# lucasbrynte/gasfm

Measured on AMD Instinct MI355X. Metric: GAT-stack edges/sec (fwd+bwd) on cam/point scene graph; 1/2/4/8 MI355X, higher is better.
Workload: dtype fp32; 1 GPU; config 4: m=1000 cameras, n=200000 points, E=4001638 projections, 12-block GraphAttnSfMNet (learning_euc widths) fwd+bwd; cameras=1000, points=200000, edges=4001638, blocks=12, parallelism=single GPU

## Files before the change

gasfm_amd/_native.py:

```python
import ctypes
import threading
import os

import numpy as np
import torch

from . import _abi
from .build import LIB

_C = _abi.constants
GASFM_OK, GASFM_ERR_INVALID, GASFM_ERR_OOM, GASFM_ERR_HIP, GASFM_ERR_UNSUPPORTED = (
    _C[k] for k in ("GASFM_OK", "GASFM_ERR_INVALID", "GASFM_ERR_OOM", "GASFM_ERR_HIP", "GASFM_ERR_UNSUPPORTED"))

_vp = ctypes.c_void_p
_i32 = ctypes.c_int32
_i64 = ctypes.c_int64

_SIGS = _abi.functions

_lib = None


def lib():
    global _lib
    if _lib is None:
        path = os.environ.get("GASFM_LIB") or LIB
        if not os.path.exists(path):
            raise ImportError(
                f"gasfm native library not built: {path} missing. Run `python -m gasfm_amd.build` "
                "(hipcc --offload-arch=gfx950). There is no CPU fallback.")
        L = ctypes.CDLL(path)
        for name, (res, args) in _SIGS.items():
            fn = getattr(L, name)
            fn.restype = res
            fn.argtypes = args
        _lib = L
    return _lib


def exported_symbols():
    return list(_SIGS)


def check(status, what):
    if status == GASFM_OK:
        return
    msg = lib().gasfm_last_error().decode(errors="replace")
    if status == GASFM_ERR_OOM:
        raise torch.OutOfMemoryError(f"{what}: {msg}")
    raise RuntimeError(f"{what} failed (status {status}): {msg}")


def _p(t):
    return None if t is None else ctypes.c_void_p(t.data_ptr())


_RAW_STREAM = getattr(torch._C, "_cuda_getCurrentRawStream", None)


def _stream(t):
    if _RAW_STREAM is not None and t.device.index is not None:
        return ctypes.c_void_p(_RAW_STREAM(t.device.index))
    return ctypes.c_void_p(torch.cuda.current_stream(t.device).cuda_stream)


def _enum(prefix):
    return {k[len(prefix):].lower(): v for k, v in _C.items() if k.startswith(prefix) and k != prefix + "COUNT"}


KERNELS = _enum("GASFM_K_")
TUNING = _enum("GASFM_TUNE_")


def dispatch_counts():
    n = _C["GASFM_K_COUNT"]
    buf = (_i64 * n)()
    lib().gasfm_dispatch_counts(buf, n)
    return {k: int(buf[i]) for k, i in KERNELS.items()}


def dispatch_reset():
    lib().gasfm_dispatch_reset()


def tuning_get(key):
    return float(lib().gasfm_tuning_get(TUNING[key]))


def tuning_set(key, value):
    check(lib().gasfm_tuning_set(TUNING[key], float(value)), "gasfm_tuning_set")


class tuned:

    def __init__(self, **kv):
        self.kv = kv

    def __enter__(self):
        self.prev = {k: tuning_get(k) for k in self.kv}
        for k, v in self.kv.items():
            tuning_set(k, v)
        return self

    def __exit__(self, *exc):
        for k, v in self.prev.items():
            tuning_set(k, v)
        return False


class dispatch_record:

    def __enter__(self):
        self.start = dispatch_counts()
        return self

    def __exit__(self, *exc):
        end = dispatch_counts()
        self.counts = {k: end[k] - self.start[k] for k in end}
        return False


def build_csr(key, n):
    key = np.ascontiguousarray(key, dtype=np.int32)
    E = key.shape[0]
    ptr = np.empty(n + 1, dtype=np.int32)
    perm = np.empty(max(E, 1), dtype=np.int32)
    st = lib().gasfm_build_csr(key.ctypes.data_as(_vp), E, n, ptr.ctypes.data_as(_vp),
                               perm.ctypes.data_as(_vp))
    check(st, "gasfm_build_csr")
    return ptr, perm[:E]


def plan_work(seg_ptr, max_piece, all_partial=False):
    seg_ptr = np.ascontiguousarray(seg_ptr, dtype=np.int32)
    N = seg_ptr.shape[0] - 1
    ni, nc, ns = _i32(0), _i32(0), _i32(0)
    L = lib()
    L.gasfm_plan_work(seg_ptr.ctypes.data_as(_vp), N, max_piece, int(all_partial), None,
                      ctypes.byref(ni), None, ctypes.byref(nc), ctypes.byref(ns))
    items = np.empty((max(ni.value, 1), 4), dtype=np.int32)
    comb = np.empty((max(nc.value, 1), 4), dtype=np.int32)
    ni2, nc2 = _i32(ni.value), _i32(nc.value)
    st = L.gasfm_plan_work(seg_ptr.ctypes.data_as(_vp), N, max_piece, int(all_partial),
                           items.ctypes.data_as(_vp), ctypes.byref(ni2), comb.ctypes.data_as(_vp),
                           ctypes.byref(nc2), ctypes.byref(ns))
    check(st, "gasfm_plan_work")
    return items[:ni2.value], comb[:nc2.value], ns.value


def attn_fwd(XL, XR, att, bias, perm, items, n_items, H, C, slope, finalize, out, seg_max, seg_sum, part=None,
             ldStat=None, lanes=False):
    ldStat = H if ldStat is None else ldStat
    fn = lib().gasfm_gat_attn_fwd_lanes if lanes else lib().gasfm_gat_attn_fwd
    st = fn(
        _p(XL), XL.stride(0), _p(XR), XR.stride(0), _p(att), _p(bias), _p(perm), _p(items), n_items, H, C,
        slope, int(finalize), _p(out), out.stride(0) if out is not None else 0, _p(seg_max), _p(seg_sum), ldStat,
        _p(part), _stream(XL))
    check(st, "gasfm_gat_attn_fwd")


def attn_combine(combine, n_combine, H, C, part, bias, finalize, out, seg_max, seg_sum, ldOut=None, ldStat=None):
    ldOut = out.stride(0) if ldOut is None else ldOut
    ldStat = H if ldStat is None else ldStat
    st = lib().gasfm_gat_attn_combine(_p(combine), n_combine, H, C, _p(part), _p(bias), int(finalize), _p(out),
                                      ldOut, _p(seg_max), _p(seg_sum), ldStat, _stream(part))
    check(st, "gasfm_gat_attn_combine")


def attn_bwd_waves(n_items, H, C):
    return lib().gasfm_gat_attn_bwd_waves(n_items, H, C)


def attn_bwd(XL, XR, att, bias, perm, items, n_items, H, C, slope, out, seg_max, seg_sum, gout, dXL, dXR,
             part_dxr, datt_part, xl_by_position=False, lanes=False):
    fn = lib().gasfm_gat_attn_bwd_lanes if lanes else lib().gasfm_gat_attn_bwd
    st = fn(
        _p(XL), XL.stride(0), _p(XR), XR.stride(0), _p(att), _p(bias), _p(perm), _p(items), n_items, H, C,
        slope, _p(out), out.stride(0), _p(seg_max), _p(seg_sum), _p(gout), gout.stride(0), _p(dXL),
        dXL.stride(0), _p(dXR), dXR.stride(0), _p(part_dxr), _p(datt_part), int(xl_by_position), _stream(dXL))
    check(st, "gasfm_gat_attn_bwd")


def attn_bwd_combine(combine, n_combine, HC, part_dxr, dXR):
    st = lib().gasfm_gat_attn_bwd_combine(_p(combine), n_combine, HC, _p(part_dxr), _p(dXR), dXR.stride(0),
                                          _stream(dXR))
    check(st, "gasfm_gat_attn_bwd_combine")


def attn_bwd_combine2(combine, n_combine, HC, part_a, out_a, part_b, out_b):
    st = lib().gasfm_gat_attn_bwd_combine2(_p(combine), n_combine, HC, _p(part_a), _p(out_a), out_a.stride(0),
                                           _p(part_b), _p(out_b), out_b.stride(0), _stream(out_a))
    check(st, "gasfm_gat_attn_bwd_combine2")


_COUNTERS = {}
_COUNTER_POOL = 1 << 16


def _counters(device, n):
    n = max(1, int(n))
    if n > _COUNTER_POOL:
        raise ValueError(f"colsum counters: {n} requested, pool holds {_COUNTER_POOL}")
    c = _COUNTERS.get(device)
    if c is None:
        c = [torch.zeros(_COUNTER_POOL, dtype=torch.int32, device=device), 0]
        _COUNTERS[device] = c
    pool, at = c
    if at + n > _COUNTER_POOL:
        at = 0
    c[1] = at + n
    return pool[at:at + n]


def colsum(A, out=None):
    assert A.dim() == 2 and A.stride(1) == 1 and A.dtype == torch.float32
    rows, cols = A.shape
    if out is None:
        out = torch.empty(cols, dtype=torch.float32, device=A.device)
    L = lib()
    ws = torch.empty(int(L.gasfm_colsum_ws_floats(rows, cols)), dtype=torch.float32, device=A.device)
    cnt = _counters(A.device, L.gasfm_colsum_counters(cols))
    st = L.gasfm_colsum(_p(A), rows, cols, max(A.stride(0), cols), _p(ws), _p(out), _p(cnt), _stream(out))
    check(st, "gasfm_colsum")
    return out


def colsum_tall_ok(A):
    return (A.dim() == 2 and A.is_contiguous() and A.dtype == torch.float32
            and bool(lib().gasfm_colsum_tall_ok(A.shape[1])))


def colsum_tall(A, out=None):
    rows, cols = A.shape
    if out is None:
        out = torch.empty(cols, dtype=torch.float32, device=A.device)
    L = lib()
    ws = torch.empty(max(1, int(L.gasfm_colsum_tall_ws_floats(rows, cols))), dtype=torch.float32, device=A.device)
    cnt = _counters(A.device, 1)
    st = L.gasfm_colsum_tall(_p(A), rows, cols, _p(ws), _p(out), _p(cnt), _stream(out))
    check(st, "gasfm_colsum_tall")
    return out


def colsum_ranges(A, row_ptr, w=None, out=None):
    if not (A.is_cuda and A.dim() == 2 and A.dtype == torch.float32 and (A.shape[1] == 1 or A.stride(1) == 1)):
        raise ValueError("colsum_ranges: A must be a 2-D fp32 CUDA tensor with unit column stride")
    rows, cols = A.shape
    if cols < 1:
        raise ValueError("colsum_ranges: A has no columns")
    if row_ptr.dtype != torch.int32 or row_ptr.dim() != 1 or row_ptr.numel() < 1 or not row_ptr.is_contiguous() \
            or row_ptr.device != A.device:
        raise ValueError("colsum_ranges: row_ptr must be a contiguous int32 vector on A's device")
    n_ranges = row_ptr.numel() - 1
    if w is not None and not (w.dtype == torch.float64 and w.dim() == 1 and w.numel() == rows and w.is_contiguous()
                              and w.device == A.device):
        raise ValueError("colsum_ranges: w must be a contiguous fp64 vector with one entry per row of A")
    if out is None:
        out = torch.empty((n_ranges, cols), dtype=torch.float64, device=A.device)
    elif not (out.dtype == torch.float64 and tuple(out.shape) == (n_ranges, cols) and out.is_contiguous()
              and out.device == A.device):
        raise ValueError(f"colsum_ranges: out must be a contiguous fp64 [{n_ranges}, {cols}] tensor")
    ld = max(A.stride(0), cols) if rows > 1 else cols
    st = lib().gasfm_colsum_ranges(_p(A), ld, cols, _p(row_ptr), n_ranges, _p(w), _p(out), _stream(out))
    check(st, "gasfm_colsum_ranges")
    return out



_DEFER_FWD = False
_PENDING = {}
_SEEN = {}
_PENDING_LOCK = threading.Lock()


def defer_token(*targets):
    if _DEFER_FWD and all(t is None or t.is_leaf for t in targets):
        return tuple(t for t in targets if t is not None) or True
    return False


class deferring_param_grads:

    def __init__(self, enabled):
        self.enabled = bool(enabled)

    def __enter__(self):
        global _DEFER_FWD
        self.prev, _DEFER_FWD = _DEFER_FWD, self.enabled
        return self

    def __exit__(self, *exc):
        global _DEFER_FWD
        _DEFER_FWD = self.prev
        return False


def param_colsum(A, defer):
    task = torch._C._current_graph_task_id() if defer else -1
    if task < 0:
        return colsum(A)
    if isinstance(defer, tuple) and any(t.grad is not None for t in defer):
        return colsum(A)
    if isinstance(defer, tuple):
        with _PENDING_LOCK:
            seen = _SEEN.setdefault(task, {})
            again = any(seen.get(id(t), id(defer)) != id(defer) for t in defer)
            for t in defer:
                seen.setdefault(id(t), id(defer))
        if again and os.environ.get("GASFM_DEBUG_DEFER"):
            print("param_colsum: repeated targets", [tuple(t.shape) for t in defer], flush=True)
        if again:
            _flush_param_colsums(task, final=False)
            return colsum(A)
    assert A.dim() == 2 and A.stride(1) == 1 and A.dtype == torch.float32
    rows, cols = A.shape
    L = lib()
    out = torch.empty(cols, dtype=torch.float32, device=A.device)
    ws = torch.empty(int(L.gasfm_colsum_ws_floats(rows, cols)), dtype=torch.float32, device=A.device)
    job = (A, ws, out, rows, cols, max(A.stride(0), cols), torch.cuda.current_stream(A.device))
    with _PENDING_LOCK:
        jobs = _PENDING.get(task)
        first = jobs is None
        if first:
            jobs = _PENDING[task] = []
        jobs.append(job)
    if first:
        torch.autograd.Variable._execution_engine.queue_callback(lambda: _flush_param_colsums(task))
    return out


def _flush_param_colsums(task, final=True):
    with _PENDING_LOCK:
        jobs = _PENDING.pop(task, [])
        if final:
            _SEEN.pop(task, None)
    if not jobs:
        return
    stream = jobs[0][6]
    assert all(j[6] == stream for j in jobs), "param_colsum: jobs queued on several streams"
    n = len(jobs)
    L = lib()
    arr = lambda ty, xs: (ty * n)(*xs)
    A = arr(ctypes.c_void_p, [j[0].data_ptr() for j in jobs])
    ws = arr(ctypes.c_void_p, [j[1].data_ptr() for j in jobs])
    out = arr(ctypes.c_void_p, [j[2].data_ptr() for j in jobs])
    rows = arr(ctypes.c_int64, [j[3] for j in jobs])
    cols = arr(ctypes.c_int32, [j[4] for j in jobs])
    ld = arr(ctypes.c_int64, [j[5] for j in jobs])
    dev = jobs[0][0].device
    cnt = _counters(dev, L.gasfm_colsum_multi_counters(n, cols))
    st = L.gasfm_colsum_multi(n, A, rows, cols, ld, ws, out, _p(cnt), ctypes.c_void_p(stream.cuda_stream))
    check(st, "gasfm_colsum_multi")


def _req(t, name, cols=None):
    if not t.is_cuda or t.dtype != torch.float32 or not t.is_contiguous():
        raise TypeError(f"{name}: expected a contiguous float32 CUDA tensor (no CPU fallback)")
    if cols is not None and t.shape[-1] != cols:
        raise ValueError(f"{name}: expected {cols} columns, got {tuple(t.shape)}")


def edge_part_floats(which, E, n_items=0):
    return lib().gasfm_edge_part_floats(which, E, n_items)


def edge_prologue_fwd(P, ln_w, ln_b, eps, W, b, Y, pos=None, W2=None, b2=None):
    _req(P, "P", 32)
    st = lib().gasfm_edge_prologue_fwd(_p(P), P.shape[0], _p(ln_w), _p(ln_b), eps, _p(W), _p(W2), _p(b), _p(b2),
                                       _p(Y), Y.stride(0), _p(pos), _stream(P))
    check(st, "gasfm_edge_prologue_fwd")


def _rows32(t, name):
    if not t.is_cuda or t.dtype != torch.float32 or t.dim() != 2 or t.shape[1] != 32 or t.stride(1) != 1 \
            or (t.shape[0] > 1 and t.stride(0) < 32):
        raise TypeError(f"{name}: expected [rows, 32] float32 CUDA rows with unit column stride")
    return t.stride(0) if t.shape[0] > 1 else 32


def edge_epilogue_fwd(P, P0, cam, pt, ln_w, ln_b, eps, Wp, bp, Sp, Sv, Sg, scale, out):
    _req(P, "P", 32)
    for t, n in ((Sp, "Sp"), (Sg, "Sg"), (Wp, "Wp")):
        _req(t, n)
    ldSv = _rows32(Sv, "Sv")
    st = lib().gasfm_edge_epilogue_fwd(_p(P), _p(P0), _p(cam), _p(pt), P.shape[0], _p(ln_w), _p(ln_b), eps, _p(Wp),
                                       Wp.shape[1], _p(bp), _p(Sp), _p(Sv), ldSv, _p(Sg), scale, _p(out),
                                       _stream(P))
    check(st, "gasfm_edge_epilogue_fwd")


def edge_epilogue_bwd(items, n_items, dPo, P, P0, ln_w, ln_b, eps, Wp, scale, dSv, part_dsv, dP0, part_w):
    _req(dPo, "dP'", 32)
    st = lib().gasfm_edge_epilogue_bwd(_p(items), n_items, _p(dPo), _p(P), _p(P0), _p(ln_w), _p(ln_b), eps, _p(Wp),
                                       Wp.shape[1], scale, _p(dSv), _p(part_dsv), _p(dP0), _p(part_w), _stream(dPo))
    check(st, "gasfm_edge_epilogue_bwd")


def edge_prologue_bwd(dXL, P, dRes, ln_w, ln_b, eps, W, Wp, scale, dP, part, W2=None, dXLc=None):
    _req(P, "P", 32)
    st = lib().gasfm_edge_prologue_bwd(_p(dXL), dXL.stride(0), _p(P), _p(dRes), P.shape[0], _p(ln_w), _p(ln_b), eps,
                                       _p(W), _p(W2), _p(Wp), Wp.shape[1] if Wp is not None else 0, scale, _p(dP),
                                       _p(part), _p(dXLc), dXLc.stride(0) if dXLc is not None else 0, _stream(P))
    check(st, "gasfm_edge_prologue_bwd")


def edge_cam_fwd(P, ln_w, ln_b, eps, Wpt, bpt, Wc, bc, XLp, pos, XR, att, bias, slope, plan_items, n_items,
                 finalize, out, seg_max, seg_sum, part, ldStat=4):
    _req(P, "P", 32)
    ldXR = _rows32(XR, "XR")
    st = lib().gasfm_edge_cam_fwd(_p(P), _p(ln_w), _p(ln_b), eps, _p(Wpt), _p(bpt), _p(Wc), _p(bc), _p(XLp),
                                  XLp.stride(0), _p(pos), _p(XR), ldXR, _p(att), _p(bias), slope, _p(plan_items),
                                  n_items, int(finalize), _p(out), out.stride(0) if out is not None else 0,
                                  _p(seg_max), _p(seg_sum), ldStat, _p(part), _stream(P))
    check(st, "gasfm_edge_cam_fwd")


def _ld_stat(seg_max):
    return seg_max.stride(0) if seg_max is not None else 4


def edge_seam_fwd(Pb, P0, pt, lnw_b, lnb_b, eps_b, Wp, bp, Sp, Sv, Sg, scale, Pout, ln_w, ln_b, eps, Wpt, bpt, Wc, bc,
                  XLp, pos, XR, att, bias, slope, plan_items, n_items, finalize, out, seg_max, seg_sum, part):
    _req(Pb, "Pb", 32)
    ldXR = _rows32(XR, "XR")
    ldSv = _rows32(Sv, "Sv")
    st = lib().gasfm_edge_seam_fwd(_p(Pb), _p(P0), _p(pt), _p(lnw_b), _p(lnb_b), eps_b, _p(Wp), Wp.stride(0), _p(bp),
                                   _p(Sp), _p(Sv), ldSv, _p(Sg), scale, _p(Pout), _p(ln_w), _p(ln_b), eps, _p(Wpt),
                                   _p(bpt), _p(Wc), _p(bc), _p(XLp), XLp.stride(0), _p(pos), _p(XR), ldXR, _p(att),
                                   _p(bias), slope, _p(plan_items), n_items, int(finalize), _p(out),
                                   out.stride(0) if out is not None else 0, _p(seg_max), _p(seg_sum), _ld_stat(seg_max),
                                   _p(part), _stream(Pb))
    check(st, "gasfm_edge_seam_fwd")


def edge0_seam_fwd(P, pt, lna_w, lna_b, lnb_w, lnb_b, eps0, Wp, bp, Wsk, bsk, Sp, Sv, Sg, scale, Pout, ln_w, ln_b, eps,
                   Wpt, bpt, Wc, bc, XLp, pos, XR, att, bias, slope, plan_items, n_items, finalize, out, seg_max,
                   seg_sum, part):
    _req(P, "P", 2)
    ldXR = _rows32(XR, "XR")
    ldSv = _rows32(Sv, "Sv")
    st = lib().gasfm_edge0_seam_fwd(_p(P), _p(pt), _p(lna_w), _p(lna_b), _p(lnb_w), _p(lnb_b), eps0, _p(Wp), _p(bp),
                                    _p(Wsk), _p(bsk), _p(Sp), _p(Sv), ldSv, _p(Sg), scale, _p(Pout), _p(ln_w), _p(ln_b),
                                    eps, _p(Wpt), _p(bpt), _p(Wc), _p(bc), _p(XLp), XLp.stride(0), _p(pos), _p(XR),
                                    ldXR, _p(att), _p(bias), slope, _p(plan_items), n_items, int(finalize), _p(out),
                                    out.stride(0) if out is not None else 0, _p(seg_max), _p(seg_sum),
                                    _ld_stat(seg_max), _p(part), _stream(P))
    check(st, "gasfm_edge0_seam_fwd")


def edge_cam_pbwd_part_shape(n_items, dwp_cols=0):
    L = lib()
    return int(L.gasfm_edge_cam_pbwd_part_rows(n_items)), int(L.gasfm_edge_cam_pbwd_part_cols()) + 32 * dwp_cols


def edge_cam_pbwd(P, ln_w, ln_b, eps, Wpt, Wc, bc, Wp, scale, XR, att, bias, slope, out, seg_max, seg_sum, gout,
                  plan_items, n_items, dXLp, dRes, dP, dXR, part_dxr, part, ldStat=4, epi=None, dwp=None):
    _req(P, "P", 32)
    ldXR = _rows32(XR, "XR")
    We = dSv = part_dsv = dP0 = None
    scale_e, ldWe = 0.0, 0
    if epi is not None:
        We, scale_e, dSv, part_dsv, dP0 = epi
        _req(dSv, "dSv", 32)
        if dP0 is not None:
            _req(dP0, "dP0", 2)
        ldWe = We.stride(0)
    P0, ldWpo = None, 0
    if dwp is not False and dwp is not None:
        P0 = dwp if isinstance(dwp, torch.Tensor) else None
        ldWpo = 34 if P0 is not None else 32
    if P0 is not None:
        _req(P0, "P0", 2)
    st = lib().gasfm_edge_cam_pbwd_ex(_p(P), _p(ln_w), _p(ln_b), eps, _p(Wpt), _p(Wc), _p(bc), _p(Wp),
                                      Wp.stride(0) if Wp is not None else 0, scale, _p(XR), ldXR, _p(att), _p(bias),
                                      slope, _p(out), out.stride(0), _p(seg_max), _p(seg_sum), ldStat, _p(gout),
                                      gout.stride(0), _p(plan_items), n_items, _p(dXLp), dXLp.stride(0), _p(dRes),
                                      _p(dP), _p(dXR), dXR.stride(0), _p(part_dxr), _p(part), part.stride(0), _p(We),
                                      ldWe, scale_e, _p(dSv), _p(part_dsv), _p(dP0), _p(P0), ldWpo, _stream(P))
    check(st, "gasfm_edge_cam_pbwd")


def segment_rowsum(items, n_items, perm, X, scale, out, part):
    st = lib().gasfm_segment_rowsum(_p(items), n_items, _p(perm), _p(X), X.stride(0), scale, _p(out), _p(part),
                                    _stream(X))
    check(st, "gasfm_segment_rowsum")


def sos_width_ok(d_in, d_out):
    return bool(lib().gasfm_sos_width_ok(int(d_in), int(d_out)))


def sos_row_tile(n_cols):
    return int(lib().gasfm_sos_row_tile(int(n_cols)))


def sos_segment_sum(plan, X, scale=1.0, mean=False, mask=None):
    _req(X, "sos_segment_sum X")
    D = X.shape[1]
    out = torch.zeros((plan.num_targets, D), dtype=torch.float32, device=X.device)
    if plan.n_items == 0 or X.shape[0] == 0:
        return out
    if mask is not None:
        _req(mask, "sos_segment_sum mask", D)
    part = torch.empty((plan.n_part_rows, D), dtype=torch.float32, device=X.device) if plan.n_part_rows else None
    st = lib().gasfm_sos_segment_sum(_p(plan.items), plan.n_items, _p(plan.perm), _p(X), X.stride(0), _p(mask),
                                     0 if mask is None else mask.stride(0), D, float(scale),
                                     _p(plan.seg_ptr) if mean else None, _p(out), _p(part), _stream(X))
    check(st, "gasfm_sos_segment_sum")
    if part is not None:
        if plan.n_l1:
            attn_bwd_combine(plan.combine_l1, plan.n_l1, D, part, part)
        if plan.n_combine:
            attn_bwd_combine(plan.combine, plan.n_combine, D, part, out)
    return out


def sos_edge_fwd(X, W, cam, pt, S, V, cmean, R, relu, out=None):
    _req(X, "sos_edge_fwd X")
    E, d_in = X.shape
    d_out = W.shape[0]
    for t, name, cols in ((W, "W", d_in), (S, "S", d_out), (V, "V", d_out)):
        _req(t, "sos_edge_fwd " + name, cols)
    Y = torch.empty((E, d_out), dtype=torch.float32, device=X.device) if out is None else out
    _req(Y, "sos_edge_fwd out", d_out)
    if Y.shape[0] != E:
        raise ValueError(f"sos_edge_fwd out: {Y.shape[0]} rows, expected {E}")
    if E == 0:
        return Y
    if cam.shape[0] != E or pt.shape[0] != E or cam.dtype != torch.int32 or pt.dtype != torch.int32:
        raise ValueError("sos_edge_fwd: cam / pt must be int32 [E]")
    if cmean is not None:
        _req(cmean, "sos_edge_fwd cmean", d_out)
    if R is not None:
        _req(R, "sos_edge_fwd R", d_out)
    st = lib().gasfm_sos_edge_fwd(_p(X), X.stride(0), _p(W), E, d_in, d_out, _p(cam), _p(pt), _p(S), _p(V),
                                  _p(cmean), _p(R), 0 if R is None else R.stride(0), int(bool(relu)), _p(Y),
                                  _stream(X))
    check(st, "gasfm_sos_edge_fwd")
    return Y


def sos_edge_dx(dY, Ym, W, cam, pt, Ac, Bp, E, d_in, out=None):
    dev = cam.device
    dX = torch.empty((E, d_in), dtype=torch.float32, device=dev) if out is None else out
    _req(dX, "sos_edge_dx out", d_in)
    if dX.shape[0] != E or cam.shape[0] != E or pt.shape[0] != E or (dY is not None and dY.shape[0] != E):
        raise ValueError("sos_edge_dx: row counts differ")
    if E == 0:
        return dX
    d_out = 0 if dY is None else dY.shape[1]
    for t, name, cols in ((dY, "dY", None), (Ym, "Ym", d_out), (W, "W", d_in), (Ac, "Ac", d_in), (Bp, "Bp", d_in)):
        if t is not None:
            _req(t, "sos_edge_dx " + name, cols)
    st = lib().gasfm_sos_edge_dx(_p(dY), _p(Ym), _p(W), E, d_in, d_out, _p(cam), _p(pt), _p(Ac), _p(Bp), _p(dX),
                                 _stream(dX))
    check(st, "gasfm_sos_edge_dx")
    return dX


def sos_edge_dw(dY, Ym, X):
    _req(dY, "sos_edge_dw dY")
    _req(X, "sos_edge_dw X")
    E, d_out = dY.shape
    d_in = X.shape[1]
    if E == 0:
        return torch.zeros((d_out, d_in), dtype=torch.float32, device=dY.device)
    if Ym is not None:
        _req(Ym, "sos_edge_dw Ym", d_out)
    L = lib()
    splits = int(L.gasfm_sos_dw_splits(E, d_in, d_out))
    part = torch.empty((splits, d_out * d_in), dtype=torch.float32, device=dY.device)
    st = L.gasfm_sos_edge_dw(_p(dY), _p(Ym), _p(X), X.stride(0), E, d_in, d_out, splits, _p(part), _stream(dY))
    check(st, "gasfm_sos_edge_dw")
    if splits == 1:
        return part.view(d_out, d_in)
    return colsum(part).view(d_out, d_in)


def edge0_part_rows(which, E, n_items=0):
    return lib().gasfm_edge0_part_rows(which, E, n_items)


def edge0_prologue_fwd(P, ln_w, ln_b, eps, W0, b0, XL, pos=None):
    _req(P, "P", 2)
    st = lib().gasfm_edge0_prologue_fwd(_p(P), P.shape[0], _p(ln_w), _p(ln_b), eps, _p(W0), _p(b0), _p(XL),
                                        _p(pos), _stream(P))
    check(st, "gasfm_edge0_prologue_fwd")


def edge0_prologue_fwd_rows(P, ln_w, ln_b, eps, W0, b0, XL, perm):
    _req(P, "P", 2)
    if perm.dtype != torch.int32 or perm.numel() != P.shape[0] or perm.device != P.device:
        raise ValueError("edge0_prologue_fwd_rows: perm must be int32 [E] on P's device")
    st = lib().gasfm_edge0_prologue_fwd_rows(_p(P), P.shape[0], _p(ln_w), _p(ln_b), eps, _p(W0), _p(b0), _p(XL),
                                             _p(perm), _stream(P))
    check(st, "gasfm_edge0_prologue_fwd_rows")


def edge0_epilogue_fwd(P, cam, pt, lna_w, lna_b, lnb_w, lnb_b, eps, Wp, bp, Wsk, bsk, Sp, Sv, Sg, scale, out):
    _req(P, "P", 2)
    for t, n in ((Sp, "Sp"), (Sg, "Sg")):
        _req(t, n)
    ldSv = _rows32(Sv, "Sv")
    st = lib().gasfm_edge0_epilogue_fwd(_p(P), _p(cam), _p(pt), P.shape[0], _p(lna_w), _p(lna_b), _p(lnb_w),
                                        _p(lnb_b), eps, _p(Wp), _p(bp), _p(Wsk), _p(bsk), _p(Sp), _p(Sv), ldSv,
                                        _p(Sg), scale, _p(out), _stream(P))
    check(st, "gasfm_edge0_epilogue_fwd")


def edge0_epilogue_bwd(items, n_items, dPo, P, lna_w, lna_b, lnb_w, lnb_b, eps, Wp, Wsk, scale, dSv, part_dsv, aux,
                       part):
    _req(dPo, "dP'", 32)
    st = lib().gasfm_edge0_epilogue_bwd(_p(items), n_items, _p(dPo), _p(P), _p(lna_w), _p(lna_b), _p(lnb_w),
                                        _p(lnb_b), eps, _p(Wp), _p(Wsk), scale, _p(dSv), _p(part_dsv), _p(aux),
                                        _p(part), _stream(dPo))
    check(st, "gasfm_edge0_epilogue_bwd")


def edge0_prologue_bwd(dXL, P, aux, ln_w, ln_b, eps, W0, dP, part):
    _req(dXL, "dXL0", 8)
    st = lib().gasfm_edge0_prologue_bwd(_p(dXL), _p(P), _p(aux), P.shape[0], _p(ln_w), _p(ln_b), eps, _p(W0),
                                        _p(dP), _p(part), _stream(P))
    check(st, "gasfm_edge0_prologue_bwd")


def node_part_rows(N, n_out, residual):
    return lib().gasfm_node_part_rows(N, n_out, int(residual))


def node_ln_linear_fwd(X, ln_w, ln_b, eps, W, b, residual, Y):
    _req(X, "X")
    N, n_in = X.shape
    st = lib().gasfm_node_ln_linear_fwd(_p(X), N, n_in, _p(ln_w), _p(ln_b), eps, _p(W), _p(b), W.shape[0],
                                        int(residual), _p(Y), Y.stride(0), _stream(X))
    check(st, "gasfm_node_ln_linear_fwd")


def node_ln_linear_bwd(dY, X, ln_w, ln_b, eps, W, residual, dX, part):
    _req(dY, "dY", W.shape[0])
    _req(X, "X")
    N, n_in = X.shape
    st = lib().gasfm_node_ln_linear_bwd(_p(dY), _p(X), N, n_in, _p(ln_w), _p(ln_b), eps, _p(W), W.shape[0],
                                        int(residual), _p(dX), _p(part), _stream(X))
    check(st, "gasfm_node_ln_linear_bwd")


def gvec_bwd_chunks(N):
    return lib().gasfm_gvec_bwd_chunks(N)


def gvec_fwd(x, ln_w, ln_b, eps, W, b, res, y):
    _req(x, "x")
    _req(W, "W")
    st = lib().gasfm_gvec_fwd(_p(x), W.shape[1], _p(ln_w), _p(ln_b), eps, _p(W), _p(b), W.shape[0], _p(res), _p(y),
                              _stream(x))
    check(st, "gasfm_gvec_fwd")


def gvec_bwd(dy, x, ln_w, ln_b, eps, W, resid, dx, dW, db, dgam, dbet, part):
    _req(dy, "dy")
    st = lib().gasfm_gvec_bwd(_p(dy), _p(x), W.shape[1], _p(ln_w), _p(ln_b), eps, _p(W), W.shape[0], int(resid),
                              _p(dx), _p(dW), _p(db), _p(dgam), _p(dbet), _p(part), _stream(x))
    check(st, "gasfm_gvec_bwd")


def point_tail_part_shape(N, has_prev):
    cols = ctypes.c_int32(0)
    rows = lib().gasfm_point_tail_part_shape(N, int(has_prev), ctypes.byref(cols))
    return rows, cols.value


def point_hub_part_shape(N, which, has_res):
    cols = ctypes.c_int32(0)
    rows = lib().gasfm_point_hub_part_shape(N, int(which), int(has_res), ctypes.byref(cols))
    return rows, cols.value


def point_tail_fwd(prev, agg, Wp, bp, ln_w, ln_b, eps, Wm, bm, out):
    _req(agg, "agg", 32)
    if prev is not None:
        _req(prev, "prev", 64)
    st = lib().gasfm_point_tail_fwd(_p(prev), _p(agg), agg.shape[0], _p(Wp), _p(bp), _p(ln_w), _p(ln_b), eps,
                                    _p(Wm), _p(bm), _p(out), _stream(agg))
    check(st, "gasfm_point_tail_fwd")


def point_tail_bwd(dout, prev, agg, Wp, bp, ln_w, ln_b, eps, Wm, dx, dagg, part):
    _req(dout, "dout", 64)
    _req(agg, "agg", 32)
    if prev is not None:
        _req(prev, "prev", 64)
    st = lib().gasfm_point_tail_bwd(_p(dout), _p(prev), _p(agg), agg.shape[0], _p(Wp), _p(bp), _p(ln_w), _p(ln_b),
                                    eps, _p(Wm), _p(dx), _p(dagg), _p(part), _stream(agg))
    check(st, "gasfm_point_tail_bwd")


def point_hub_fwd(X, eps, gA, bA, WA, SA, WB, bB, XL, gC, bC, WC, bWC, WD, bD, XR):
    _req(X, "X", 64)
    st = lib().gasfm_point_hub_fwd(_p(X), X.shape[0], eps, _p(gA), _p(bA), _p(WA), _p(SA), _p(WB), _p(bB), _p(XL),
                                   _p(gC), _p(bC), _p(WC), _p(bWC), _p(WD), _p(bD), _p(XR), _stream(X))
    check(st, "gasfm_point_hub_fwd")


def point_tail_hub_fwd(prev, agg, Wp, bp, ln_w, ln_b, eps, Wm, bm, out, eps_h, gA, bA, WA, SA, WB, bB, XL, gC, bC,
                       WC, bWC, WD, bD, XR):
    _req(agg, "agg", 32)
    _req(out, "out", 64)
    if prev is not None:
        _req(prev, "prev", 64)
    st = lib().gasfm_point_tail_hub_fwd(_p(prev), _p(agg), agg.shape[0], _p(Wp), _p(bp), _p(ln_w), _p(ln_b), eps,
                                        _p(Wm), _p(bm), _p(out), eps_h, _p(gA), _p(bA), _p(WA), _p(SA), _p(WB), _p(bB),
                                        _p(XL), _p(gC), _p(bC), _p(WC), _p(bWC), _p(WD), _p(bD), _p(XR), _stream(agg))
    check(st, "gasfm_point_tail_hub_fwd")


def point_hub_bwd(X, eps, gA, bA, WA, WB, gC, bC, WC, bWC, WD, dSA, dXL, dXR, dRes, dX, part_a, part_c):
    _req(X, "X", 64)
    _req(dSA, "dSA", 32)
    _req(dXL, "dXL", 64)
    _req(dXR, "dXR", 32)
    if dRes is not None:
        _req(dRes, "dRes", 64)
    st = lib().gasfm_point_hub_bwd(_p(X), X.shape[0], eps, _p(gA), _p(bA), _p(WA), _p(WB), _p(gC), _p(bC), _p(WC),
                                   _p(bWC), _p(WD), _p(dSA), _p(dXL), _p(dXR), _p(dRes), _p(dX), _p(part_a),
                                   _p(part_c), _stream(X))
    check(st, "gasfm_point_hub_bwd")


def embed2_fwd(X, W, b, Y):
    _req(X, "values", 2)
    _req(Y, "P", 2)
    st = lib().gasfm_embed2_fwd(_p(X), X.shape[0], _p(W), _p(b), _p(Y), _stream(X))
    check(st, "gasfm_embed2_fwd")


def embed2_bwd(X, dY, defer=False):
    _req(X, "values", 2)
    _req(dY, "dP", 2)
    E = X.shape[0]
    rows = lib().gasfm_embed2_part_rows(E)
    if rows == 0:
        tot = torch.zeros(6, dtype=torch.float32, device=X.device)
    else:
        part = torch.empty((rows, 6), dtype=torch.float32, device=X.device)
        st = lib().gasfm_embed2_bwd(_p(X), _p(dY), E, _p(part), _stream(X))
        check(st, "gasfm_embed2_bwd")
        tot = param_colsum(part, defer)
    return tot[:4].view(2, 2), tot[4:]


def point_head_part_shape(N, which):
    cols = ctypes.c_int32(0)
    rows = lib().gasfm_point_head_part_shape(N, int(which), ctypes.byref(cols))
    return rows, cols.value


def _head_weights(W1, b1, W2, b2, W3, b3=None):
    shapes = ((W1, (64, 64)), (b1, (64,)), (W2, (64, 64)), (b2, (64,)), (W3, (3, 64))) + \
        (((b3, (3,)),) if b3 is not None else ())
    for t, shape in shapes:
        if tuple(t.shape) != shape or not t.is_contiguous() or t.dtype != torch.float32:
            raise ValueError(f"point head: weight {tuple(t.shape)} is not a contiguous fp32 {shape}")


def point_head_fwd(P, W1, b1, W2, b2, W3, b3, out):
    _req(P, "P", 64)
    _head_weights(W1, b1, W2, b2, W3, b3)
    N = P.shape[0]
    if tuple(out.shape) != (4, N) or not out.is_contiguous():
        raise ValueError("point_head_fwd: out must be a contiguous [4, N]")
    st = lib().gasfm_point_head_fwd(_p(P), N, _p(W1), _p(b1), _p(W2), _p(b2), _p(W3), _p(b3), _p(out), _stream(P))
    check(st, "gasfm_point_head_fwd")


def point_head_bwd(P, W1, b1, W2, b2, W3, dout, dP, part_a, part_b):
    _req(P, "P", 64)
    _req(dP, "dP", 64)
    _head_weights(W1, b1, W2, b2, W3)
    N = P.shape[0]
    if tuple(dout.shape) != (4, N) or not dout.is_contiguous():
        raise ValueError("point_head_bwd: dout must be a contiguous [4, N]")
    for part, which in ((part_a, 0), (part_b, 1)):
        if tuple(part.shape) != point_head_part_shape(N, which) or not part.is_contiguous():
            raise ValueError("point_head_bwd: partial buffer of the wrong shape")
    st = lib().gasfm_point_head_bwd(_p(P), N, _p(W1), _p(b1), _p(W2), _p(b2), _p(W3), _p(dout), _p(dP),
                                    _p(part_a), _p(part_b), _stream(P))
    check(st, "gasfm_point_head_bwd")


def view_tail_part_cols(D):
    return lib().gasfm_view_tail_part_cols(D)


def view_hub_part_cols(D):
    return lib().gasfm_view_hub_part_cols(D)


def view_scratch(m, D, device):
    return torch.empty(max(1, int(lib().gasfm_view_scratch_floats(m, D))), dtype=torch.float32, device=device)


def view_tail_fwd(prev, agg, Wp, bp, ln_w, ln_b, eps, bm, x, xb, h, rs, scratch):
    _req(agg, "agg", 32)
    D = x.shape[1]
    if prev is not None:
        _req(prev, "prev", D)
    st = lib().gasfm_view_tail_fwd(_p(prev), _p(agg), agg.shape[0], D, _p(Wp), _p(bp), _p(ln_w), _p(ln_b), eps,
                                   _p(bm), _p(x), _p(xb), _p(h), _p(rs), _p(scratch), _stream(agg))
    check(st, "gasfm_view_tail_fwd")


def view_tail_bwd(dv, dh, x, rs, agg, Wp, ln_w, ln_b, dx, dagg, part, scratch):
    D = x.shape[1]
    for t, n in ((dv, "dv"), (dh, "dh"), (x, "x")):
        _req(t, n, D)
    _req(agg, "agg", 32)
    st = lib().gasfm_view_tail_bwd(_p(dv), _p(dh), _p(x), _p(rs), _p(agg), agg.shape[0], D, _p(Wp), _p(ln_w),
                                   _p(ln_b), _p(dx), _p(dagg), _p(part), _p(scratch), _stream(agg))
    check(st, "gasfm_view_tail_bwd")


def view_hub_fwd(v, eps, gC, bC, Wv, gA, bA, Wa, ba, Wr, br, sv, t, xr, rs, scratch):
    _req(v, "v")
    ldo = _rows32(sv, "sv")
    if _rows32(xr, "xr") != ldo:
        raise ValueError("view_hub_fwd: sv and xr need the same row stride")
    st = lib().gasfm_view_hub_fwd(_p(v), v.shape[0], v.shape[1], eps, _p(gC), _p(bC), _p(Wv), _p(gA), _p(bA), _p(Wa),
                                  _p(ba), _p(Wr), _p(br), _p(sv), _p(t), _p(xr), ldo, _p(rs), _p(scratch), _stream(v))
    check(st, "gasfm_view_hub_fwd")


def view_chain_ok(m, D):
    return bool(lib().gasfm_view_chain_ok(m, D))


def _vc_scratch(m, D, device):
    return torch.empty(max(1, int(lib().gasfm_view_chain_scratch_floats(m, D))), dtype=torch.float32, device=device)


def view_chain_tail_fwd(prev, agg, Wp, bp, ln_w, ln_b, eps, Wm, bm, view, x, h, rs):
    _req(agg, "agg", 32)
    m, D = view.shape
    for t, n in ((view, "view"), (x, "x"), (h, "h"), (Wm, "Wm"), (Wp, "Wp")) + (((prev, "prev"),) if prev is not None else ()):
        _req(t, n)
    st = lib().gasfm_view_chain_tail_fwd(_p(prev), _p(agg), m, D, _p(Wp), _p(bp), _p(ln_w), _p(ln_b), eps, _p(Wm),
                                         _p(bm), _p(view), _p(x), _p(h), _p(rs), _stream(agg))
    check(st, "gasfm_view_chain_tail_fwd")


def view_chain_hub_fwd(v, eps, Wl, bl, gC, bC, Wv, gA, bA, Wa, ba, Wr, br, XL, sv, t, xr, rs):
    _req(v, "v")
    ldo = _rows32(sv, "sv")
    if _rows32(xr, "xr") != ldo:
        raise ValueError("view_chain_hub_fwd: sv and xr need the same row stride")
    for a, n in ((Wl, "Wl"), (Wv, "Wv"), (Wa, "Wa"), (XL, "XL")):
        _req(a, n)
    st = lib().gasfm_view_chain_hub_fwd(_p(v), v.shape[0], v.shape[1], eps, _p(Wl), _p(bl), _p(gC), _p(bC), _p(Wv),
                                        _p(gA), _p(bA), _p(Wa), _p(ba), _p(Wr), _p(br), _p(XL), _p(sv), _p(t), _p(xr),
                                        ldo, _p(rs), _stream(v))
    check(st, "gasfm_view_chain_hub_fwd")


def view_chain_hub_bwd(v, rs, gC, bC, Wv, gA, bA, Wa, t, Wr, Wl, dsv, dxr, dxl, dres, dacc, dWl, part):
    _req(v, "v")
    m, D = v.shape
    for a, n, w in ((t, "t", 32), (dsv, "dsv", 32), (dxr, "dxr", 32), (dxl, "dxl", D), (dacc, "dacc", D),
                    (dWl, "dWl", D)):
        _req(a, n, w)
    if dres is not None:
        _req(dres, "dres", D)
    scratch = _vc_scratch(m, D, v.device)
    st = lib().gasfm_view_chain_hub_bwd(_p(v), _p(rs), m, D, _p(gC), _p(bC), _p(Wv), _p(gA), _p(bA), _p(Wa), _p(t),
                                        _p(Wr), _p(Wl), _p(dsv), _p(dxr), _p(dxl), _p(dres), _p(dacc), _p(dWl),
                                        _p(part), _p(scratch), _stream(v))
    check(st, "gasfm_view_chain_hub_bwd")


def view_chain_tail_bwd(dv, x, h, rs, agg, Wp, ln_w, ln_b, Wm, dh, dWm, dx, dagg, part):
    m, D = x.shape
    for a, n in ((dv, "dv"), (x, "x"), (h, "h"), (dh, "dh"), (dx, "dx"), (dWm, "dWm")):
        _req(a, n, D)
    _req(agg, "agg", 32)
    scratch = _vc_scratch(m, D, x.device)
    cnt = _counters(x.device, lib().gasfm_view_chain_counters(m))
    st = lib().gasfm_view_chain_tail_bwd(_p(dv), _p(x), _p(h), _p(rs), _p(agg), m, D, _p(Wp), _p(ln_w), _p(ln_b),
                                         _p(Wm), _p(dh), _p(dWm), _p(dx), _p(dagg), _p(part), _p(scratch), _p(cnt),
                                         _stream(x))
    check(st, "gasfm_view_chain_tail_bwd")


def view_hub_bwd(v, rs, gC, bC, Wv, gA, bA, Wa, t, Wr, dsv, dxr, dxl, dacc, part, scratch, dres=None):
    _req(v, "v")
    D = v.shape[1]
    for a, n, w in ((t, "t", 32), (dsv, "dsv", 32), (dxr, "dxr", 32), (dxl, "dxl", D), (dacc, "dacc", D)):
        _req(a, n, w)
    if dres is not None:
        _req(dres, "dres", D)
    st = lib().gasfm_view_hub_bwd(_p(v), _p(rs), v.shape[0], D, _p(gC), _p(bC), _p(Wv), _p(gA), _p(bA), _p(Wa),
                                  _p(t), _p(Wr), _p(dsv), _p(dxr), _p(dxl), _p(dres), _p(dacc), _p(part),
                                  _p(scratch), _stream(v))
    check(st, "gasfm_view_hub_bwd")


def pose_fwd(x, P):
    if not x.is_cuda or x.dtype != torch.float32 or x.stride(1) != 1:
        raise TypeError("pose x: expected a float32 CUDA tensor with unit column stride (no CPU fallback)")
    check(lib().gasfm_pose_fwd(_p(x), x.stride(0), x.shape[0], _p(P), _stream(x)), "gasfm_pose_fwd")


def pose_bwd(x, dP, dx):
    _req(dP, "dP")
    check(lib().gasfm_pose_bwd(_p(x), x.stride(0), x.shape[0], _p(dP), _p(dx), dx.stride(0), _stream(x)),
          "gasfm_pose_bwd")


def _i32vec(t, name):
    if not t.is_cuda or t.dtype != torch.int32 or t.dim() != 1 or not t.is_contiguous():
        raise TypeError(f"{name}: expected a contiguous int32 CUDA vector")


def _edge_args(name, cam, pt, vals, P, X, csr=None, seg=None, scene_of=None, f32=()):
    vecs = [(cam, "cam"), (pt, "pt")]
    if csr is not None:
        vecs += [(csr[0], "cam_ptr"), (csr[1], "pt_ptr")] + ([] if csr[2] is None else [(csr[2], "perm")])
    if scene_of is not None:
        vecs += [(scene_of[0], "scene_of_cam"), (scene_of[1], "scene_of_pt")]
    for t, tname in vecs:
        _i32vec(t, f"{name}: {tname}")
    for t, tname, cols in ((vals, "vals", 2), (P, "P", 12), (X, "pts3D", None)) + tuple(f32):
        _req(t, f"{name}: {tname}", cols)
    if X.dim() != 2 or X.shape[0] != 4 or P.dim() != 2 or vals.dim() != 2:
        raise ValueError(f"{name}: expected P [m, 12], pts3D [4, n] and vals [E, 2]")
    E, m, n = cam.shape[0], P.shape[0], X.shape[1]
    if pt.shape[0] != E or vals.shape[0] != E:
        raise ValueError(f"{name}: expected pts3D [4, n] and E-long cam / pt / values")
    if csr is not None and (csr[0].shape[0] != m + 1 or csr[1].shape[0] != n + 1
                            or (csr[2] is not None and csr[2].shape[0] != E)):
        raise ValueError(f"{name}: CSR shapes do not match m / n / E")
    if scene_of is not None and (scene_of[0].shape[0] != m or scene_of[1].shape[0] != n):
        raise ValueError(f"{name}: scene map shapes do not match m / n")
    if seg is not None:
        eoff, S = seg
        if not eoff.is_cuda or eoff.dtype != torch.int32 or not eoff.is_contiguous() or eoff.numel() != S + 1:
            raise TypeError(f"{name}: eoff must be a contiguous int32 [S + 1] CUDA tensor")
    return E, m, n


def _grad_args(dloss, dP, dX, n, tot=None):
    return ((dloss, "dloss", None), (dP, "dP", 12), (dX, "dX", n)) + (() if tot is None else ((tot, "tot", None),))


def esfm_part_rows(E):
    return lib().gasfm_esfm_part_rows(E)


def esfm_fwd(cam, pt, vals, P, X, margin, hinge_w, hinge, part):
    E, _, n = _edge_args("esfm_fwd", cam, pt, vals, P, X)
    st = lib().gasfm_esfm_fwd(_p(cam), _p(pt), _p(vals), E, _p(P), _p(X), n, margin, hinge_w, int(hinge), _p(part),
                              _stream(X))
    check(st, "gasfm_esfm_fwd")


def esfm_bwd(cptr, pptr, perm, cam, pt, vals, P, X, margin, hinge_w, hinge, equalize, valid_only, dloss, tot, dP,
             dX, E_norm=None):
    E, m, n = _edge_args("esfm_bwd", cam, pt, vals, P, X, csr=(cptr, pptr, perm),
                         f32=_grad_args(dloss, dP, dX, X.shape[-1], tot))
    E_norm = E if E_norm is None else int(E_norm)
    st = lib().gasfm_esfm_bwd(_p(cptr), m, _p(pptr), _p(perm), _p(cam), _p(pt), _p(vals), E, E_norm, _p(P), _p(X), n,
                              margin, hinge_w, int(hinge), int(equalize), int(valid_only), _p(dloss), _p(tot), _p(dP),
                              _p(dX), _stream(X))
    check(st, "gasfm_esfm_bwd")


def esfm_seg_fwd(cam, pt, vals, eoff, weight, P, X, margin, hinge_w, hinge):
    S = int(weight.numel())
    _, _, n = _edge_args("esfm_seg_fwd", cam, pt, vals, P, X, seg=(eoff, S), f32=((weight, "weight", None),))
    dev = X.device
    part = torch.empty((lib().gasfm_esfm_seg_part_rows(S), 2), dtype=torch.float32, device=dev)
    tot = torch.empty((S, 2), dtype=torch.float32, device=dev)
    loss = torch.empty(1, dtype=torch.float32, device=dev)
    st = lib().gasfm_esfm_seg_fwd(_p(cam), _p(pt), _p(vals), _p(eoff), S, _p(weight), _p(P), _p(X), n, margin, hinge_w,
                                  int(hinge), _p(part), _p(tot), _p(loss), _stream(X))
    check(st, "gasfm_esfm_seg_fwd")
    return loss, tot


def esfm_seg_bwd(cptr, pptr, perm, cam, pt, vals, eoff, scene_of_cam, scene_of_pt, weight, P, X, margin, hinge_w,
                 hinge, equalize, valid_only, dloss, tot, dP, dX):
    S = int(weight.numel())
    _, m, n = _edge_args("esfm_seg_bwd", cam, pt, vals, P, X, csr=(cptr, pptr, perm), seg=(eoff, S),
                         scene_of=(scene_of_cam, scene_of_pt),
                         f32=((weight, "weight", None),) + _grad_args(dloss, dP, dX, X.shape[-1], tot))
    st = lib().gasfm_esfm_seg_bwd(_p(cptr), m, _p(pptr), _p(perm), _p(cam), _p(pt), _p(vals), _p(eoff), S,
                                  _p(scene_of_cam), _p(scene_of_pt), _p(weight), _p(P), _p(X), n, margin, hinge_w,
                                  int(hinge), int(equalize), int(valid_only), _p(dloss), _p(tot), _p(dP), _p(dX),
                                  _stream(X))
    check(st, "gasfm_esfm_seg_bwd")


def ose_fwd(cam, pt, vals, P, X, w_reg):
    E, _, n = _edge_args("ose_fwd", cam, pt, vals, P, X)
    part = torch.empty((lib().gasfm_ose_part_rows(E), 1), dtype=torch.float32, device=X.device)
    st = lib().gasfm_ose_fwd(_p(cam), _p(pt), _p(vals), E, _p(P), _p(X), n, w_reg, _p(part), _stream(X))
    check(st, "gasfm_ose_fwd")
    return part


def ose_bwd(cptr, pptr, perm, cam, pt, vals, P, X, w_reg, dloss, dP, dX):
    E, m, n = _edge_args("ose_bwd", cam, pt, vals, P, X, csr=(cptr, pptr, perm),
                         f32=_grad_args(dloss, dP, dX, X.shape[-1]))
    st = lib().gasfm_ose_bwd(_p(cptr), m, _p(pptr), _p(perm), _p(cam), _p(pt), _p(vals), E, _p(P), _p(X), n, w_reg,
                             _p(dloss), _p(dP), _p(dX), _stream(X))
    check(st, "gasfm_ose_bwd")


def ose_seg_fwd(cam, pt, vals, eoff, weight, P, X, w_reg):
    S = int(weight.numel())
    _, _, n = _edge_args("ose_seg_fwd", cam, pt, vals, P, X, seg=(eoff, S), f32=((weight, "weight", None),))
    dev = X.device
    part = torch.empty(lib().gasfm_ose_seg_part_rows(S), dtype=torch.float32, device=dev)
    tot = torch.empty(S, dtype=torch.float32, device=dev)
    loss = torch.empty(1, dtype=torch.float32, device=dev)
    st = lib().gasfm_ose_seg_fwd(_p(cam), _p(pt), _p(vals), _p(eoff), S, _p(weight), _p(P), _p(X), n, w_reg, _p(part),
                                 _p(tot), _p(loss), _stream(X))
    check(st, "gasfm_ose_seg_fwd")
    return loss, tot


def ose_seg_bwd(cptr, pptr, perm, cam, pt, vals, eoff, scene_of_cam, scene_of_pt, weight, P, X, w_reg, dloss, dP, dX):
    S = int(weight.numel())
    _, m, n = _edge_args("ose_seg_bwd", cam, pt, vals, P, X, csr=(cptr, pptr, perm), seg=(eoff, S),
                         scene_of=(scene_of_cam, scene_of_pt),
                         f32=((weight, "weight", None),) + _grad_args(dloss, dP, dX, X.shape[-1]))
    st = lib().gasfm_ose_seg_bwd(_p(cptr), m, _p(pptr), _p(perm), _p(cam), _p(pt), _p(vals), _p(eoff), S,
                                 _p(scene_of_cam), _p(scene_of_pt), _p(weight), _p(P), _p(X), n, w_reg, _p(dloss),
                                 _p(dP), _p(dX), _stream(X))
    check(st, "gasfm_ose_seg_bwd")


def reproj_error(cam, pt, xy, P, X, err=None):
    E, _, n = _edge_args("reproj_error", cam, pt, xy, P, X, f32=() if err is None else ((err, "err", None),))
    if err is not None and err.shape[0] != E:
        raise ValueError("reproj_error: expected pts3D [4, n] and E-long cam / pt / xy / err")
    part = torch.empty((esfm_part_rows(E), 2), dtype=torch.float32, device=X.device)
    st = lib().gasfm_reproj_error(_p(cam), _p(pt), _p(xy), E, _p(P), _p(X), n, _p(err), _p(part), _stream(X))
    check(st, "gasfm_reproj_error")
    return part


def reproj_error_seg(cam, pt, xy, eoff, S, P, X):
    _, _, n = _edge_args("reproj_error_seg", cam, pt, xy, P, X, seg=(eoff, S))
    dev = X.device
    part = torch.empty((lib().gasfm_esfm_seg_part_rows(S), 2), dtype=torch.float32, device=dev)
    tot = torch.empty((S, 2), dtype=torch.float32, device=dev)
    st = lib().gasfm_reproj_error_seg(_p(cam), _p(pt), _p(xy), _p(eoff), S, _p(P), _p(X), n, _p(part), _p(tot),
                                      _stream(X))
    check(st, "gasfm_reproj_error_seg")
    return tot


def depth_stats(cam, pt, cam_ptr, pt_ptr, perm, P, X, margin, depth=None):
    E, m, n = cam.shape[0], cam_ptr.shape[0] - 1, pt_ptr.shape[0] - 1
    for t, name in ((cam, "cam"), (pt, "pt"), (cam_ptr, "cam_ptr"), (pt_ptr, "pt_ptr")):
        _i32vec(t, name)
    if perm is not None:
        _i32vec(perm, "perm")
    _req(P, "P", 12), _req(X, "pts3D", n)
    if (X.dim() != 2 or X.shape[0] != 4 or P.dim() != 2 or P.shape[0] != m or pt.shape[0] != E
            or (perm is not None and perm.shape[0] != E) or (depth is not None and depth.shape[0] != E)):
        raise ValueError("depth_stats: expected P [m, 12], pts3D [4, n], cam_ptr [m + 1], pt_ptr [n + 1] and "
                         "E-long cam / pt / perm / depth")
    if depth is not None:
        _req(depth, "depth")
    dev = cam_ptr.device
    cam_neg = torch.empty(m, dtype=torch.int32, device=dev)
    pt_neg = torch.empty(n, dtype=torch.int32, device=dev)
    stats = torch.empty(6, dtype=torch.float64, device=dev)
    L = lib()
    ws = torch.empty(int(L.gasfm_depth_stats_ws_doubles(E)), dtype=torch.float64, device=dev)
    st = L.gasfm_depth_stats(_p(cam), _p(pt), E, _p(cam_ptr), m, _p(pt_ptr), _p(perm), n, _p(P), _p(X),
                             float(margin), _p(depth), _p(cam_neg), _p(pt_neg), _p(ws), _p(stats), _stream(cam_ptr))
    check(st, "gasfm_depth_stats")
    return cam_neg, pt_neg, stats


def _depth_args(a, b, name):
    _req(a, "depths"), _req(b, "depth targets")
    if a.dim() != 1 or a.shape != b.shape or a.shape[0] == 0:
        raise ValueError(f"{name}: expected two non-empty [E] vectors, got {tuple(a.shape)}, {tuple(b.shape)}")


def depth_loss_fwd(a, b, l2):
    _depth_args(a, b, "depth_loss_fwd")
    E, L = a.shape[0], lib()
    part = torch.empty((L.gasfm_depth_loss_part_rows(E), 2), dtype=torch.float32, device=a.device)
    check(L.gasfm_depth_loss_sums(_p(a), _p(b), E, _p(part), _stream(a)), "gasfm_depth_loss_sums")
    sums = colsum(part)
    part = torch.empty_like(part)
    check(L.gasfm_depth_loss_fwd(_p(a), _p(b), E, _p(sums), int(l2), _p(part), _stream(a)), "gasfm_depth_loss_fwd")
    return sums, colsum(part)


def depth_loss_bwd(a, b, sums, tot, l2, dloss):
    _depth_args(a, b, "depth_loss_bwd")
    _req(dloss, "dloss")
    da = torch.empty_like(a)
    st = lib().gasfm_depth_loss_bwd(_p(a), _p(b), a.shape[0], _p(sums), _p(tot), int(l2), _p(dloss), _p(da),
                                    _stream(a))
    check(st, "gasfm_depth_loss_bwd")
    return da


UnionScene = _abi.structs["gasfm_union_scene"]
UnionOut = _abi.structs["gasfm_union_out"]
UnionPad = _abi.structs["gasfm_union_pad"]


def union_fill_scene(sc, out, stream_of):
    check(lib().gasfm_union_fill_scene(ctypes.byref(sc), ctypes.byref(out), _stream(stream_of)),
          "gasfm_union_fill_scene")


def fold_scene_rows_fwd(sv, sg, soc):
    out = torch.empty((sv.shape[0], sv.shape[1]), dtype=torch.float32, device=sv.device)
    check(lib().gasfm_fold_scene_rows_fwd(_p(sv), sv.stride(0), _p(sg), sg.stride(0), _p(soc), sv.shape[0],
                                          sv.shape[1], _p(out), out.stride(0), _stream(sv)), "gasfm_fold_scene_rows_fwd")
    return out


def fold_scene_rows_bwd(dout, soc, S):
    dsg = torch.empty((S, dout.shape[1]), dtype=torch.float32, device=dout.device)
    check(lib().gasfm_fold_scene_rows_bwd(_p(dout), dout.stride(0), _p(soc), dout.shape[0], S, dout.shape[1], _p(dsg),
                                          dsg.stride(0), _stream(dout)), "gasfm_fold_scene_rows_bwd")
    return dsg


ADAM_CHUNK = _C["GASFM_ADAM_CHUNK"]


def adam_step(tensors, chunks, n_chunks, lr, beta1, beta2, eps, weight_decay, step, stream_of):
    check(lib().gasfm_adam_step(_p(tensors), _p(chunks), int(n_chunks), float(lr), float(beta1), float(beta2),
                                float(eps), float(weight_decay), int(step), _stream(stream_of)), "gasfm_adam_step")


CLIP_MODES = {None: _C["GASFM_CLIP_NONE"], "norm": _C["GASFM_CLIP_NORM"], "value": _C["GASFM_CLIP_VALUE"]}
ADAM_CTL_FLOATS = ctypes.sizeof(_abi.structs["gasfm_adam_ctl"]) // 4


def grad_sumsq(tensors, chunks, n_chunks, partial, stream_of):
    check(lib().gasfm_grad_sumsq(_p(tensors), _p(chunks), int(n_chunks), _p(partial), _stream(stream_of)),
          "gasfm_grad_sumsq")


def grad_sumsq_finish(partial, n, total, norm):
    check(lib().gasfm_grad_sumsq_finish(_p(partial), int(n), _p(total), _p(norm), _stream(total)),
          "gasfm_grad_sumsq_finish")


def grad_clip(tensors, chunks, n_chunks, mode, threshold, norm, stream_of):
    check(lib().gasfm_grad_clip(_p(tensors), _p(chunks), int(n_chunks), CLIP_MODES[mode], float(threshold), _p(norm),
                                _stream(stream_of)), "gasfm_grad_clip")


def adam_control(ctl, sumsq, loss, lr, step, beta1, beta2, clip_mode, clip_th):
    lr_dev = lr if torch.is_tensor(lr) else None
    check(lib().gasfm_adam_control(_p(ctl), _p(sumsq), _p(loss), _p(lr_dev), 0.0 if lr_dev is not None else float(lr),
                                   _p(step), float(beta1), float(beta2), CLIP_MODES[clip_mode], float(clip_th or 0.0),
                                   _stream(ctl)), "gasfm_adam_control")


def adam_step_ctl(tensors, chunks, n_chunks, ctl, beta1, beta2, eps, weight_decay, clip_mode, clip_th):
    check(lib().gasfm_adam_step_ctl(_p(tensors), _p(chunks), int(n_chunks), _p(ctl), float(beta1), float(beta2),
                                    float(eps), float(weight_decay), CLIP_MODES[clip_mode], float(clip_th or 0.0),
                                    _stream(ctl)), "gasfm_adam_step_ctl")


def union_fill_pad(pd, out, stream_of):
    check(lib().gasfm_union_fill_pad(ctypes.byref(pd), ctypes.byref(out), _stream(stream_of)), "gasfm_union_fill_pad")


_SOS_TABLES_IN = ("cam_ptr", "pt_ptr", "soc32", "sop32", "cam32", "eoff")
_SOS_TABLES_I32 = ("ptrc", "ptrp", "ptre")
_SOS_TABLES_F64 = ("Es", "degc", "invc", "wc", "degp", "invp", "wp")
_SOS_TABLES_I64 = ("sop", "soe")


SosTables = _abi.structs["gasfm_sos_tables"]


def sos_tables_args(cam_ptr, pt_ptr, soc32, sop32, cam32, eoff, out):
    M, N, E, S = soc32.numel(), sop32.numel(), cam32.numel(), eoff.numel() - 1
    dev = soc32.device
    want = dict(cam_ptr=M + 1, pt_ptr=N + 1, soc32=M, sop32=N, cam32=E, eoff=S + 1, ptrc=S + 1, ptrp=S + 1,
                ptre=S + 1, Es=S, degc=M, invc=M, wc=M, degp=N, invp=N, wp=N, sop=N, soe=E)
    given = dict(cam_ptr=cam_ptr, pt_ptr=pt_ptr, soc32=soc32, sop32=sop32, cam32=cam32, eoff=eoff)
    if S < 1 or M < 1 or N < 1:
        raise ValueError(f"sos_union_tables: S={S} M={M} N={N}")
    t = SosTables()
    for group, dtype in ((_SOS_TABLES_IN, torch.int32), (_SOS_TABLES_I32, torch.int32),
                         (_SOS_TABLES_F64, torch.float64), (_SOS_TABLES_I64, torch.int64)):
        for k in group:
            v = given[k] if k in given else getattr(out, k)
            if not (v.is_cuda and v.device == dev and v.dtype == dtype and v.dim() == 1 and v.is_contiguous()
                    and v.numel() == want[k]):
                raise ValueError(f"sos_union_tables: {k} must be a contiguous {dtype} CUDA vector of {want[k]} entries")
            setattr(t, k, v.data_ptr())
    t.M, t.N, t.E, t.S = M, N, E, S
    return t


def sos_union_tables(t, stream_of):
    check(lib().gasfm_sos_union_tables(ctypes.byref(t), _stream(stream_of)), "gasfm_sos_union_tables")


def _ptrs(ts):
    return (ctypes.c_void_p * len(ts))(*[None if t is None else t.data_ptr() for t in ts])


def _ints(v):
    return (ctypes.c_int32 * len(v))(*v)


def gvec_multi_fwd(probs, eps):
    cols = list(zip(*probs))
    for W in cols[3]:
        _req(W, "W")
    K = [W.shape[1] for W in cols[3]]
    N = [W.shape[0] for W in cols[3]]
    st = lib().gasfm_gvec_multi_fwd(len(probs), *[_ptrs(c) for c in cols], _ints(K), _ints(N), eps,
                                    _stream(cols[0][0]))
    check(st, "gasfm_gvec_multi_fwd")


def gvec_multi_bwd(probs, groups, eps):
    dy, x, lw, lb, W, dW, db, dg, dbt, part = (list(c) for c in zip(*probs))
    K = [w.shape[1] for w in W]
    N = [w.shape[0] for w in W]
    p0, npr, dres, dx = (list(c) for c in zip(*groups))
    st = lib().gasfm_gvec_multi_bwd(len(probs), _ptrs(dy), _ptrs(x), _ptrs(lw), _ptrs(lb), _ptrs(W), _ints(K),
                                    _ints(N), _ptrs(dW), _ptrs(db), _ptrs(dg), _ptrs(dbt), _ptrs(part), len(groups),
                                    _ints(p0), _ints(npr), _ptrs(dres), _ptrs(dx), eps, _stream(x[0]))
    check(st, "gasfm_gvec_multi_bwd")


_GC_W = ("W1", "b1", "gM", "bM", "W2", "b2", "gA", "bA", "WA", "gB", "bB", "WB", "bWB", "gC", "bC", "WC", "bWC",
         "WD", "bD", "WE", "bE")
_GC_D = tuple("d" + k for k in _GC_W)


_GC_SHADOW = ("W1", "W2", "WA", "WB", "WC", "WD", "WE")


_GChain = _abi.structs["gasfm_gchain"]
_GChainGrads = _abi.structs["gasfm_gchain_grads"]
GCHAIN_MAX_ROWS = _C["GASFM_GCHAIN_MAX_ROWS"]


def gchain_struct(w, eps_m, eps_h, shadows=None, rows=1):
    c = _GChain()
    W1, WA = w["W1"], w["WA"]
    hub = w.get("WB") is not None
    dims = dict(G=W1.shape[0], Kc=W1.shape[1], NA=WA.shape[0], NB=w["WB"].shape[0] if hub else 0,
                NC=w["WC"].shape[0] if hub else 0, ND=w["WD"].shape[0] if hub else 0,
                NE=w["WE"].shape[0] if hub else 0)
    for k, v in dims.items():
        setattr(c, k, int(v))
    c.eps_m, c.eps_h = float(eps_m), float(eps_h)
    for k in _GC_W:
        t = w.get(k)
        if t is not None:
            _req(t, k)
            setattr(c, k, t.data_ptr())
    for k, t in (shadows or {}).items():
        if t is not None:
            if t.dtype != torch.bfloat16 or not t.is_contiguous() or t.shape != w[k].shape:
                raise ValueError(f"gchain: the bf16 shadow of {k} must be a contiguous bf16 tensor of its shape")
            setattr(c, k + "h", t.data_ptr())
    if not 1 <= rows <= GCHAIN_MAX_ROWS:
        raise ValueError(f"gchain: {rows} rows (1..{GCHAIN_MAX_ROWS})")
    c.rows = int(rows)
    return c


def gchain_fwd(c, xcat, prev, x1, g, sg, xv, xp, xrv, xrp):
    st = lib().gasfm_gchain_fwd(ctypes.addressof(c), _p(xcat), _p(prev), _p(x1), _p(g), _p(sg), _p(xv), _p(xp),
                                _p(xrv), _p(xrp), _stream(g))
    check(st, "gasfm_gchain_fwd")


def gchain_bwd(c, xcat, x1, g, xv, xp, dskip, dsg, dxrv, dxrp, dxcat, dprev, grads):
    d = _GChainGrads()
    for k in _GC_D:
        t = grads.get(k)
        if t is not None:
            setattr(d, k, t.data_ptr())
    L = lib()
    ws = torch.empty(int(L.gasfm_gchain_scratch_floats(ctypes.addressof(c))), dtype=torch.float32, device=g.device)
    cnt = _counters(g.device, L.gasfm_gchain_counters(ctypes.addressof(c)))
    st = L.gasfm_gchain_bwd(ctypes.addressof(c), _p(xcat), _p(x1), _p(g), _p(xv), _p(xp), _p(dskip), _p(dsg),
                            _p(dxrv), _p(dxrp), _p(dxcat), _p(dprev), ctypes.addressof(d), _p(ws), _p(cnt),
                            _stream(g))
    check(st, "gasfm_gchain_bwd")


_GattProb = _abi.structs["gasfm_gatt_prob"]


def _gatt_probs(probs):
    arr = (_GattProb * len(probs))()
    for q, d in enumerate(probs):
        XL = d["XL"]
        if not XL.is_cuda or XL.dtype != torch.float32 or XL.stride(1) != 1:
            raise TypeError("gatt: XL must be a float32 CUDA tensor with unit column stride")
        src = d.get("src")
        if src is not None and (src.dtype != torch.int32 or not src.is_contiguous()):
            raise TypeError("gatt: src must be a contiguous int32 tensor")
        a = arr[q]
        a.XL, a.ldXL, a.src, a.S, a.HC = XL.data_ptr(), XL.stride(0), _p(src), int(d["S"]), int(d["att"].numel())
        for k in ("XR", "att", "bias", "out", "smax", "ssum", "part", "gout", "dXR", "datt"):
            setattr(a, k, _p(d.get(k)))
        dXL = d.get("dXL")
        if dXL is not None:
            if dXL.stride(1) != 1:
                raise TypeError("gatt: dXL must have unit column stride")
            a.dXL, a.ldDXL = dXL.data_ptr(), dXL.stride(0)
    return arr


def gatt_fwd(probs, slope):
    arr = _gatt_probs(probs)
    L = lib()
    dev = probs[0]["XL"].device
    ws = torch.empty(int(L.gasfm_gatt_scratch_floats(len(probs), ctypes.addressof(arr))), dtype=torch.float32, device=dev)
    cnt = _counters(dev, int(L.gasfm_gatt_counters(len(probs), ctypes.addressof(arr))))
    check(L.gasfm_gatt_fwd(len(probs), ctypes.addressof(arr), float(slope), _p(ws), _p(cnt), _stream(probs[0]["XL"])),
          "gasfm_gatt_fwd")


def gatt_bwd(probs, slope):
    arr = _gatt_probs(probs)
    L = lib()
    dev = probs[0]["XL"].device
    ws = torch.empty(int(L.gasfm_gatt_scratch_floats(len(probs), ctypes.addressof(arr))), dtype=torch.float32, device=dev)
    cnt = _counters(dev, int(L.gasfm_gatt_counters(len(probs), ctypes.addressof(arr))))
    check(L.gasfm_gatt_bwd(len(probs), ctypes.addressof(arr), float(slope), _p(ws), _p(cnt), _stream(probs[0]["XL"])),
          "gasfm_gatt_bwd")


def gatt_merge(probs, nrows, stride, unpack=None):
    arr = (_GattProb * len(probs))()
    for q, d in enumerate(probs):
        a = arr[q]
        a.HC = int(d["bias"].numel())
        for k in ("bias", "out", "smax", "ssum", "part"):
            setattr(a, k, _p(d[k]))
    if unpack is None:
        check(lib().gasfm_gatt_merge(len(probs), ctypes.addressof(arr), int(nrows), int(stride), _stream(d["bias"])),
              "gasfm_gatt_merge")
        return
    G, blk, roff, chunk, dst = unpack
    _exchange_args(G, dst, None)
    check(lib().gasfm_gatt_merge_unpack(len(probs), ctypes.addressof(arr), int(nrows), int(stride), _p(G), int(nrows),
                                        int(blk), int(roff), int(chunk), int(dst.shape[1]), int(dst.shape[0]), _p(dst),
                                        dst.stride(0) if dst.shape[0] > 1 else dst.shape[1], _stream(G)),
          "gasfm_gatt_merge_unpack")


def _exchange_args(G, rows_dst, sum_dst):
    for t, nm in ((G, "G"), (rows_dst, "rows_dst"), (sum_dst, "sum_dst")):
        if t is not None and (not t.is_cuda or t.dtype != torch.float32 or t.stride(-1) != 1):
            raise TypeError(f"exchange_unpack: {nm} must be float32 CUDA with unit column stride")


def exchange_unpack(G, W, blk, rows=None, sums=None):
    roff, chunk, rdst = rows if rows is not None else (0, 1, None)
    soff, sdst = sums if sums is not None else (0, None)
    _exchange_args(G, rdst, sdst)
    width = int(rdst.shape[1]) if rdst is not None else 4
    m = int(rdst.shape[0]) if rdst is not None else 0
    ld = (rdst.stride(0) if m > 1 else width) if rdst is not None else 4
    check(lib().gasfm_exchange_unpack(_p(G), int(W), int(blk), int(roff), int(chunk), width, m, _p(rdst), ld,
                                      int(soff), int(sdst.numel()) if sdst is not None else 0, _p(sdst), _stream(G)),
          "gasfm_exchange_unpack")


def scan_i32(x):
    _i32vec(x, "scan input")
    out = torch.empty(x.shape[0] + 1, dtype=torch.int32, device=x.device)
    check(lib().gasfm_scan_i32(_p(x), x.shape[0], _p(out), _stream(x)), "gasfm_scan_i32")
    return out


def _dev_check(what, *ts):
    for name, t, dt in ts:
        if t is not None and (not t.is_cuda or t.dtype != dt or not t.is_contiguous()):
            raise TypeError(f"{what}: {name} must be a contiguous {dt} CUDA tensor")


def outlier_counts(state, cam_ptr, pt_ptr, perm, m, n):
    _dev_check("outlier_counts", ("state", state, torch.uint8), ("cam_ptr", cam_ptr, torch.int32),
               ("pt_ptr", pt_ptr, torch.int32), ("perm", perm, torch.int32))
    if cam_ptr.shape[0] != m + 1 or pt_ptr.shape[0] != n + 1:
        raise ValueError("outlier_counts: cam_ptr / pt_ptr must have m + 1 / n + 1 entries")
    dev = state.device
    cam_in = torch.empty(m, dtype=torch.int32, device=dev)
    pt_in = torch.empty(n, dtype=torch.int32, device=dev)
    mins = torch.empty(2, dtype=torch.int32, device=dev)
    check(lib().gasfm_outlier_counts(_p(state), _p(cam_ptr), _p(pt_ptr), _p(perm), m, n, _p(cam_in), _p(pt_in),
                                     _p(mins), _stream(state)), "gasfm_outlier_counts")
    return cam_in, pt_in, mins


def outlier_mark(state, cam, pt, cam_in, pt_in, mode, counts=None):
    _dev_check("outlier_mark", ("state", state, torch.uint8), ("cam", cam, torch.int64), ("pt", pt, torch.int64),
               ("cam_in", cam_in, torch.int32), ("pt_in", pt_in, torch.int32))
    E = state.shape[0]
    if cam.shape[0] != E or pt.shape[0] != E:
        raise ValueError("outlier_mark: cam / pt must have one entry per edge")
    if counts is None:
        counts = torch.empty(4, dtype=torch.int32, device=state.device)
    check(lib().gasfm_outlier_mark(_p(state), _p(cam), _p(pt), _p(cam_in), _p(pt_in), E, mode, _p(counts),
                                   _stream(state)), "gasfm_outlier_mark")
    return counts


def outlier_moments(values, state, cam_ptr, m):
    _dev_check("outlier_moments", ("values", values, torch.float32), ("state", state, torch.uint8),
               ("cam_ptr", cam_ptr, torch.int32))
    if values.dim() != 2 or values.shape[1] != 2 or values.shape[0] != state.shape[0] or cam_ptr.shape[0] != m + 1:
        raise ValueError("outlier_moments: values [E, 2], state [E], cam_ptr [m + 1]")
    dev = values.device
    mu = torch.empty((m, 2), dtype=torch.float32, device=dev)
    sigma = torch.empty((m, 2, 2), dtype=torch.float32, device=dev)
    tril = torch.empty((m, 2, 2), dtype=torch.float32, device=dev)
    piv = torch.empty((m, 2), dtype=torch.int32, device=dev)
    check(lib().gasfm_outlier_moments(_p(values), _p(state), _p(cam_ptr), m, _p(mu), _p(sigma), _p(tril), _p(piv),
                                      _stream(values)), "gasfm_outlier_moments")
    return mu, sigma, tril, piv


def outlier_apply(idx, cam, pt, z, mu, tril, M, pix=None):
    _dev_check("outlier_apply", ("idx", idx, torch.int64), ("cam", cam, torch.int64), ("pt", pt, torch.int64),
               ("z", z, torch.float32), ("mu", mu, torch.float32), ("scale_tril", tril, torch.float32),
               ("pix", pix, torch.float32))
    _check_M(M, "outlier_apply")
    k = idx.shape[0]
    if z.numel() != 2 * k:
        raise ValueError(f"outlier_apply: z has {z.numel()} values for {k} outliers")
    m = M.shape[0] // 2
    if mu.shape != (m, 2) or tril.shape != (m, 2, 2):
        raise ValueError("outlier_apply: mu [m, 2], scale_tril [m, 2, 2]")
    check(lib().gasfm_outlier_apply(_p(idx), k, _p(cam), _p(pt), _p(z), _p(mu), _p(tril), _p(M), M.stride(0),
                                    _p(pix), _stream(M)), "gasfm_outlier_apply")


def _check_M(M, what):
    if not M.is_cuda or M.dtype != torch.float32 or M.dim() != 2 or M.stride(1) != 1 or M.shape[0] % 2:
        raise TypeError(f"{what}: M must be a float32 CUDA [2m, n] matrix with unit column stride "
                        "(no CPU fallback)")


def scene_mask(M):
    _check_M(M, "scene_mask")
    m, n = M.shape[0] // 2, M.shape[1]
    L = lib()
    dev = M.device
    W, T = L.gasfm_scene_mask_words(n), L.gasfm_scene_tiles(m, n)
    i32 = dict(dtype=torch.int32, device=dev)
    mask = torch.empty(m * W, dtype=torch.int64, device=dev)
    pt_valid = torch.empty(W, dtype=torch.int64, device=dev)
    view_count, pt_count = torch.empty(n, **i32), torch.empty(n, **i32)
    tile_count, tile_base = torch.empty(T, **i32), torch.empty(T + 1, **i32)
    check(L.gasfm_scene_mask(_p(M), M.stride(0), m, n, _p(mask), _p(view_count), _p(pt_valid), _p(pt_count),
                             _p(tile_count), _p(tile_base), _stream(M)), "gasfm_scene_mask")
    return mask, pt_valid, pt_count, tile_base


def scene_homography(M, Ns, R, Ninv):
    _check_M(M, "scene_homography")
    m, n = M.shape[0] // 2, M.shape[1]
    for t, name in ((Ns, "Ns"), (R, "R"), (Ninv, "Ninv")):
        if not t.is_cuda or t.dtype != torch.float32 or tuple(t.shape) != (m, 3, 3) or not t.is_contiguous():
            raise TypeError(f"scene_homography: {name} must be a contiguous float32 CUDA [m, 3, 3] tensor")
    mask, pt_valid, _, _ = scene_mask(M)
    out = torch.empty_like(M)
    check(lib().gasfm_scene_homography(_p(M), M.stride(0), m, n, _p(mask), _p(pt_valid), _p(Ns), _p(R), _p(Ninv),
                                       _p(out), out.stride(0), _stream(M)), "gasfm_scene_homography")
    return out


def scene_build(M, Ns=None):
    _check_M(M, "scene_build")
    m, n = M.shape[0] // 2, M.shape[1]
    if Ns is not None:
        if not Ns.is_cuda or Ns.dtype != torch.float32 or tuple(Ns.shape) != (m, 3, 3):
            raise TypeError("scene_build: Ns must be a float32 CUDA [m, 3, 3] tensor")
        Ns = Ns.contiguous()
    L = lib()
    dev = M.device
    T = L.gasfm_scene_tiles(m, n)
    i32 = dict(dtype=torch.int32, device=dev)
    mask, pt_valid, pt_count, tile_base = scene_mask(M)
    st = _stream(M)
    W = L.gasfm_scene_mask_words(n)
    E = int(tile_base[T].item())
    cam = torch.empty(E, dtype=torch.int64, device=dev)
    pt = torch.empty(E, dtype=torch.int64, device=dev)
    vals = torch.empty((E, 2), dtype=torch.float32, device=dev)
    word_base = torch.empty(m * W, **i32)
    check(L.gasfm_scene_emit(_p(M), M.stride(0), _p(Ns) if Ns is not None else None, m, n, _p(mask), _p(pt_valid),
                             _p(tile_base), _p(cam), _p(pt), _p(vals), _p(word_base), st), "gasfm_scene_emit")
    pt_ptr = scan_i32(pt_count)
    perm, pos = torch.empty(E, **i32), torch.empty(E, **i32)
    if E:
        check(L.gasfm_scene_point_csr(_p(mask), _p(pt_valid), _p(word_base), _p(pt_ptr), m, n, _p(perm), _p(pos),
                                      st), "gasfm_scene_point_csr")
    cam_ptr = tile_base[0::T // m].contiguous() if T else torch.zeros(m + 1, **i32)
    return {"cam": cam, "pt": pt, "values": vals, "pt_count": pt_count, "cam_ptr": cam_ptr, "pt_ptr": pt_ptr,
            "perm": perm, "pos": pos}


def _edge_ids(t, name, what):
    if not t.is_cuda or t.dtype not in (torch.int32, torch.int64) or t.dim() != 1 or not t.is_contiguous():
        raise TypeError(f"{what}: {name} must be a contiguous int32 or int64 CUDA vector")
    return t, int(t.dtype == torch.int64)


def scene_shard_bounds(pt_ptr, world):
    _dev_check("scene_shard_bounds", ("pt_ptr", pt_ptr, torch.int32))
    if world < 1 or pt_ptr.dim() != 1 or pt_ptr.shape[0] < 1:
        raise ValueError("scene_shard_bounds: world >= 1 and pt_ptr [n + 1]")
    bounds = torch.empty(world + 1, dtype=torch.int32, device=pt_ptr.device)
    check(lib().gasfm_scene_shard_bounds(_p(pt_ptr), pt_ptr.shape[0] - 1, world, _p(bounds), _stream(pt_ptr)),
          "gasfm_scene_shard_bounds")
    return bounds


def scene_shard_ranges(cam_ptr, pt_ptr, pt, bounds, rank, c0=0, c1=0):
    what = "scene_shard_ranges"
    _dev_check(what, ("cam_ptr", cam_ptr, torch.int32), ("pt_ptr", pt_ptr, torch.int32), ("bounds", bounds, torch.int32))
    pt, is64 = _edge_ids(pt, "pt", what)
    m, n = cam_ptr.shape[0] - 1, pt_ptr.shape[0] - 1
    if m < 0 or n < 0 or not 0 <= rank < bounds.shape[0] - 1 or not 0 <= c0 <= c1 <= m:
        raise ValueError(f"{what}: rank {rank} of {bounds.shape[0] - 1}, cameras [{c0}, {c1}) of {m}")
    dev = cam_ptr.device
    L, st = lib(), _stream(cam_ptr)
    lo = torch.empty(m, dtype=torch.int32, device=dev)
    count = torch.empty(m, dtype=torch.int32, device=dev)
    ppc = torch.empty(m, dtype=torch.int64, device=dev)
    vv = torch.empty(m, dtype=torch.uint8, device=dev)
    stats = torch.empty(9, dtype=torch.int64, device=dev)
    check(L.gasfm_scene_shard_cam_range(_p(cam_ptr), _p(pt), is64, m, _p(bounds), rank, _p(lo), _p(count), _p(ppc),
                                        _p(vv), st), "gasfm_scene_shard_cam_range")
    check(L.gasfm_scene_shard_stats(_p(cam_ptr), m, _p(pt_ptr), n, _p(bounds), rank, c0, c1, _p(stats), st),
          "gasfm_scene_shard_stats")
    return {"lo": lo, "count": count, "lcam_ptr": scan_i32(count), "pts_per_cam": ppc, "valid_view": vv.view(torch.bool),
            "stats": stats}


def scene_shard_emit(r, pt, p0, E_loc, sources):
    what = "scene_shard_emit"
    pt, is64 = _edge_ids(pt, "pt", what)
    if len(sources) > 3:
        raise ValueError(f"{what}: at most three source arrays")
    for s in sources:
        if not s.is_cuda or s.dtype != torch.float32 or s.dim() != 2 or s.shape != (pt.shape[0], 2) \
                or not s.is_contiguous():
            raise TypeError(f"{what}: sources must be contiguous float32 CUDA [E, 2] arrays")
    dev = pt.device
    m = r["lo"].shape[0]
    sel = torch.empty(E_loc, dtype=torch.int64, device=dev)
    indices = torch.empty((2, E_loc), dtype=torch.int64, device=dev)
    cam32 = torch.empty(E_loc, dtype=torch.int32, device=dev)
    pt32 = torch.empty(E_loc, dtype=torch.int32, device=dev)
    dst = [torch.empty((E_loc, 2), dtype=torch.float32, device=dev) for _ in sources]
    sp = [_p(s) for s in sources] + [None] * (3 - len(sources))
    dp = [_p(d) for d in dst] + [None] * (3 - len(dst))
    check(lib().gasfm_scene_shard_emit(_p(r["lcam_ptr"]), _p(r["lo"]), m, _p(pt), is64, E_loc, p0, sp[0], sp[1], sp[2],
                                       _p(sel), _p(indices), _p(cam32), _p(pt32), dp[0], dp[1], dp[2], _stream(pt)),
          "gasfm_scene_shard_emit")
    return sel, indices, cam32, pt32, dst


def scene_shard_point_csr(r, pt_ptr, perm, cam, p0, p1, E_loc):
    what = "scene_shard_point_csr"
    _dev_check(what, ("pt_ptr", pt_ptr, torch.int32), ("perm", perm, torch.int32))
    cam, is64 = _edge_ids(cam, "cam", what)
    n_loc = p1 - p0
    if not 0 <= p0 <= p1 < pt_ptr.shape[0] or (perm is not None and perm.shape[0] != cam.shape[0]):
        raise ValueError(f"{what}: points [{p0}, {p1}) of {pt_ptr.shape[0] - 1}; perm must have one entry per edge")
    dev = cam.device
    i32 = dict(dtype=torch.int32, device=dev)
    lpt_ptr = torch.empty(n_loc + 1, **i32)
    cpp = torch.empty(n_loc, dtype=torch.int64, device=dev)
    vp = torch.empty(n_loc, dtype=torch.uint8, device=dev)
    lperm, lpos = torch.empty(E_loc, **i32), torch.empty(E_loc, **i32)
    check(lib().gasfm_scene_shard_point_csr(_p(pt_ptr), _p(perm), _p(cam), is64, _p(r["lcam_ptr"]), _p(r["lo"]), p0,
                                            n_loc, E_loc, _p(lpt_ptr), _p(cpp), _p(vp), _p(lperm), _p(lpos),
                                            _stream(cam)), "gasfm_scene_shard_point_csr")
    return lpt_ptr, cpp, vp.view(torch.bool), lperm, lpos


def _depth_edges(what, cam, pt):
    cam, is64 = _edge_ids(cam, "cam", what)
    pt, pis64 = _edge_ids(pt, "pt", what)
    if is64 != pis64 or cam.shape != pt.shape:
        raise TypeError(f"{what}: cam and pt must have one dtype and one length")
    return cam, pt, is64


def _depth_part(E, dev):
    part = torch.empty(int(lib().gasfm_depth_part_slots(E)), dtype=torch.int32, device=dev)
    return part, torch.zeros(1, dtype=torch.int32, device=dev)


def depth_targets(a, X, cam, pt, out=None):
    what = "depth_targets"
    cam, pt, is64 = _depth_edges(what, cam, pt)
    for t, name in ((a, "a"), (X, "X")):
        if not t.is_cuda or t.dtype != torch.float32 or t.dim() != 2 or t.shape[1] != 4 or not t.is_contiguous():
            raise TypeError(f"{what}: {name} must be a contiguous float32 CUDA [rows, 4] tensor")
    E = cam.shape[0]
    d = torch.empty(E, dtype=torch.float32, device=cam.device) if out is None else out
    _dev_check(what, ("out", d, torch.float32))
    if d.shape != (E,):
        raise ValueError(f"{what}: out must have one entry per edge")
    part, bad = _depth_part(E, cam.device)
    check(lib().gasfm_depth_targets(_p(a), a.shape[0], _p(X), X.shape[0], _p(cam), _p(pt), is64, E, _p(d), _p(part),
                                    _p(bad), _stream(cam)), "gasfm_depth_targets")
    return d, bad


def depth_gather(pcam_ptr, ppt, pd, view_idx, keep, cam, pt, out=None):
    what = "depth_gather"
    cam, pt, is64 = _depth_edges(what, cam, pt)
    ppt, pis64 = _edge_ids(ppt, "parent pt", what)
    _dev_check(what, ("parent cam_ptr", pcam_ptr, torch.int32), ("parent depths", pd, torch.float32),
               ("view_idx", view_idx, torch.int64), ("keep", keep, torch.int64))
    if pcam_ptr.dim() != 1 or pcam_ptr.shape[0] < 1 or pd.shape != ppt.shape or view_idx.dim() != 1 or keep.dim() != 1:
        raise ValueError(f"{what}: parent cam_ptr [m + 1], parent pt / depths [E], view_idx [m'], keep [n']")
    E = cam.shape[0]
    d = torch.empty(E, dtype=torch.float32, device=cam.device) if out is None else out
    _dev_check(what, ("out", d, torch.float32))
    if d.shape != (E,):
        raise ValueError(f"{what}: out must have one entry per edge")
    part, missing = _depth_part(E, cam.device)
    check(lib().gasfm_depth_gather(_p(pcam_ptr), _p(ppt), pis64, _p(pd), pcam_ptr.shape[0] - 1, ppt.shape[0],
                                   _p(view_idx), _p(keep), view_idx.shape[0], keep.shape[0], _p(cam), _p(pt), is64, E,
                                   _p(d), _p(part), _p(missing), _stream(cam)), "gasfm_depth_gather")
    return d, missing


def depth_rescale(d, cam, pt, M, Ns, R, out=None):
    what = "depth_rescale"
    _check_M(M, what)
    cam, pt, is64 = _depth_edges(what, cam, pt)
    m, n = M.shape[0] // 2, M.shape[1]
    for t, name in ((Ns, "Ns"), (R, "R")):
        if not t.is_cuda or t.dtype != torch.float32 or tuple(t.shape) != (m, 3, 3) or not t.is_contiguous():
            raise TypeError(f"{what}: {name} must be a contiguous float32 CUDA [m, 3, 3] tensor")
    _dev_check(what, ("d", d, torch.float32))
    E = cam.shape[0]
    res = torch.empty(E, dtype=torch.float32, device=cam.device) if out is None else out
    _dev_check(what, ("out", res, torch.float32))
    if d.shape != (E,) or res.shape != (E,):
        raise ValueError(f"{what}: d and out must have one entry per edge")
    check(lib().gasfm_depth_rescale(_p(d), _p(cam), _p(pt), is64, E, _p(M), M.stride(0), m, n, _p(Ns), _p(R), _p(res),
                                    _stream(cam)), "gasfm_depth_rescale")
    return res


def sum_n(tensors):
    t0 = tensors[0]
    for t in tensors:
        _req(t, "sum_n input")
        if t.shape != t0.shape:
            raise ValueError("sum_n: shapes differ")
    if t0.numel() % 4:
        out = tensors[0].clone()
        for t in tensors[1:]:
            out += t
        return out
    out = torch.empty_like(t0)
    st = lib().gasfm_sum_n(len(tensors), _ptrs(tensors), t0.numel(), _p(out), _stream(t0))
    check(st, "gasfm_sum_n")
    return out


def _gemm(fn, what, a, b, cin=None, bias=None, out=None):
    for t, nm in ((a, what + " a"), (b, what + " b")):
        if not (t.is_cuda and t.dtype == torch.float32 and t.dim() == 2):
            raise ValueError(f"{nm}: fp32 CUDA matrix required")
    M, K = a.shape
    K2, N = b.shape
    if K2 != K:
        raise ValueError(f"{what}: inner dimensions {K} and {K2} differ")
    if out is None:
        out = torch.empty((M, N), dtype=torch.float32, device=a.device)
    if cin is not None and (cin.shape != (M, N) or cin.stride(1) != 1):
        raise ValueError(f"{what}: cin must be [M, N] with unit column stride")
    if bias is not None and (bias.shape != (N,) or not bias.is_contiguous()):
        raise ValueError(f"{what}: bias must be a contiguous [N] vector")
    if out.shape != (M, N) or out.stride(1) != 1:
        raise ValueError(f"{what}: out must be [M, N] with unit column stride")
    st = fn(M, N, K, _p(a), a.stride(0), a.stride(1), _p(b), b.stride(0), b.stride(1), _p(cin),
            cin.stride(0) if cin is not None else 0, _p(bias), _p(out), out.stride(0), _stream(out))
    check(st, what)
    return out


def gemm_bf16(a, b, cin=None, bias=None, out=None):
    return _gemm(lib().gasfm_gemm_bf16, "gasfm_gemm_bf16", a, b, cin, bias, out)


def gemm_f32_smallm(a, b, cin=None, bias=None, out=None):
    if not (a.is_cuda and b.is_cuda and a.dtype == torch.float32 and b.dtype == torch.float32
            and a.dim() == 2 and b.dim() == 2 and a.shape[1] == b.shape[0]):
        return None
    M, K = a.shape
    N = b.shape[1]
    L = lib()
    if a.stride(1) == 1 and a.stride(0) % 4 == 0:
        if b.stride(0) == 1 and b.stride(1) % 4 == 0:
            mode, A, lda, B, ldb = 0, a, a.stride(0), b, b.stride(1)
        elif b.stride(1) == 1 and cin is None and bias is None:
            mode, A, lda, B, ldb = 1, a, a.stride(0), b, b.stride(0)
        else:
            return None
        I, J = M, N
    elif a.stride(0) == 1 and b.stride(1) == 1 and cin is None and bias is None:
        mode, A, lda, B, ldb = 2, a, a.stride(1), b, b.stride(0)
        I, J = M, N
    else:
        return None
    if mode in (0, 1) and (A.data_ptr() % 16 or (mode == 0 and B.data_ptr() % 16)):
        return None
    if not L.gasfm_gemm_f32_smallm_ok(mode, I, J, K):
        return None
    if out is None:
        out = torch.empty((M, N), dtype=torch.float32, device=a.device)
    if out.shape != (M, N) or out.stride(1) != 1 or (cin is not None and (cin.shape != (M, N) or cin.stride(1) != 1)):
        return None
    if bias is not None and (bias.shape != (N,) or not bias.is_contiguous()):
        return None
    st = L.gasfm_gemm_f32_smallm(mode, I, J, K, _p(A), lda, _p(B), ldb, _p(bias), _p(cin),
                                 cin.stride(0) if cin is not None else 0, _p(out), out.stride(0), _stream(out))
    check(st, "gasfm_gemm_f32_smallm")
    return out


def gemm_f32(a, b, cin=None, bias=None, out=None):
    return _gemm(lib().gasfm_gemm_f32, "gasfm_gemm_f32", a, b, cin, bias, out)
```

gasfm_amd/build.py:

```python
import glob
import os
import subprocess
import sys

HERE = os.path.dirname(os.path.abspath(__file__))
CSRC = os.path.join(HERE, "csrc")
LIB = os.path.join(HERE, "libgasfm.so")
HEADER = os.path.join(HERE, "..", "include", "gasfm.h")
DEPTH_HEAD_HEADER = os.path.join(HERE, "..", "include", "gasfm_depth_head.h")
ARCH = os.environ.get("GASFM_OFFLOAD_ARCH", "gfx950")


def sources():
    return sorted(glob.glob(os.path.join(CSRC, "*.hip")) + glob.glob(os.path.join(CSRC, "*.cpp")))


def file_flags(src):
    with open(src) as f:
        first = f.readline()
    tag = "// hipcc-flags:"
    return first[len(tag):].split() if first.startswith(tag) else []


def _stale():
    if not os.path.exists(LIB):
        return True
    t = os.path.getmtime(LIB)
    deps = sources() + glob.glob(os.path.join(CSRC, "*.hpp")) + [HEADER, DEPTH_HEAD_HEADER]
    return any(os.path.getmtime(p) > t for p in deps if os.path.exists(p))


def build(force=False, verbose=False, defines=(), out=None):
    lib = out or LIB
    if out is None and not force and not _stale():
        return LIB
    hipcc = os.environ.get("HIPCC", "/opt/rocm/bin/hipcc")
    objs = []
    tag = "" if out is None else "_" + os.path.splitext(os.path.basename(out))[0]
    build_dir = os.path.join(HERE, "_build" + tag)
    os.makedirs(build_dir, exist_ok=True)
    procs = []
    for src in sources():
        obj = os.path.join(build_dir, os.path.basename(src) + ".o")
        cmd = [hipcc, f"--offload-arch={ARCH}", "-O3", "-fPIC", "-std=c++17", "-c", src, "-o", obj] + file_flags(src)
        cmd += [f"-D{d}" for d in defines]
        if verbose:
            print(" ".join(cmd), file=sys.stderr)
        procs.append((src, subprocess.Popen(cmd, stdout=subprocess.PIPE, stderr=subprocess.STDOUT)))
        objs.append(obj)
    for src, p in procs:
        out, _ = p.communicate()
        if p.returncode != 0:
            raise RuntimeError(f"hipcc failed on {src}:\n{out.decode(errors='replace')}")
    tmp = lib + ".tmp"
    cmd = [hipcc, f"--offload-arch={ARCH}", "-shared", "-fPIC", "-o", tmp] + objs
    r = subprocess.run(cmd, stdout=subprocess.PIPE, stderr=subprocess.STDOUT)
    if r.returncode != 0:
        raise RuntimeError("link failed:\n" + r.stdout.decode(errors="replace"))
    os.replace(tmp, lib)
    return lib


if __name__ == "__main__":
    print(build(force="--force" in sys.argv, verbose=True))
```

gasfm_amd/csrc/global_chain.hip:

```cpp
#include <hip/hip_runtime.h>

#include <cstdint>

#include "common.hpp"

namespace gasfm {
namespace {

constexpr int kFT = 256;
constexpr int kBT = 256;
constexpr int kSW = 32;
constexpr int kMaxK = 2048;
constexpr int kPer = kMaxK / 256;
constexpr int kMaxProb = 3;
constexpr int kMaxRaw = 3;
constexpr int kMaxRows = GASFM_GCHAIN_MAX_ROWS;

__device__ __forceinline__ float wave_sum(float v) {
#pragma unroll
  for (int o = 32; o > 0; o >>= 1) v += __shfl_xor(v, o);
  return v;
}

template <int NV>
__device__ __forceinline__ void block_sums(float (&v)[NV], float* scratch) {
  const int lane = threadIdx.x & 63, wave = threadIdx.x >> 6;
#pragma unroll
  for (int k = 0; k < NV; ++k) v[k] = wave_sum(v[k]);
  __syncthreads();
  if (lane == 0) {
#pragma unroll
    for (int k = 0; k < NV; ++k) scratch[wave * NV + k] = v[k];
  }
  __syncthreads();
#pragma unroll
  for (int k = 0; k < NV; ++k) v[k] = scratch[k] + scratch[NV + k] + scratch[2 * NV + k] + scratch[3 * NV + k];
}

template <bool BF>
__device__ __forceinline__ float4 w4(const float* W, const uint16_t* Wh, int64_t off) {
  if (BF) {
    const uint2 t = *reinterpret_cast<const uint2*>(Wh + off);
    return make_float4(__uint_as_float(t.x << 16), __uint_as_float(t.x & 0xffff0000u), __uint_as_float(t.y << 16),
                       __uint_as_float(t.y & 0xffff0000u));
  }
  return *reinterpret_cast<const float4*>(W + off);
}

__device__ __forceinline__ void row_stats(const float (&xv)[kPer], int K, float eps, float* scratch, float& mean,
                                          float& rstd) {
  float s[1] = {0.f};
#pragma unroll
  for (int u = 0; u < kPer; ++u) s[0] += xv[u];
  block_sums<1>(s, scratch);
  mean = s[0] / K;
  float q[1] = {0.f};
#pragma unroll
  for (int u = 0; u < kPer; ++u) {
    const int j = int(threadIdx.x) + 256 * u;
    const float d = j < K ? xv[u] - mean : 0.f;
    q[0] = fmaf(d, d, q[0]);
  }
  block_sums<1>(q, scratch);
  rstd = rsq_normal(q[0] / K + eps);
}

__device__ __forceinline__ void load_row(const float* __restrict__ x, int K, float (&xv)[kPer]) {
#pragma unroll
  for (int u = 0; u < kPer; ++u) {
    const int j = int(threadIdx.x) + 256 * u;
    xv[u] = j < K ? x[j] : 0.f;
  }
}

template <int NP>
__device__ __forceinline__ int find_prob(const int (&blk0)[NP], int nprob) {
  int pi = 0;
  while (pi + 1 < nprob && int(blockIdx.x) >= blk0[pi + 1]) ++pi;
  return pi;
}

struct GnFwdProb {
  const float* x;
  const float* gam;
  const float* bet;
  const float* W;
  const float* b;
  const float* res;
  float* y;
  int K, N, blk0;
  float eps;
  const uint16_t* Wh;
  int rows;
};
struct GnFwdArgs {
  GnFwdProb p[kMaxProb];
  int nprob;
};

template <int KI, bool BF, int R>
__global__ __launch_bounds__(kFT) void gnode_fwd_kernel(GnFwdArgs a) {
  __shared__ __attribute__((aligned(16))) float h[kMaxK];
  __shared__ float scratch[8];
  int blk0[kMaxProb];
#pragma unroll
  for (int q = 0; q < kMaxProb; ++q) blk0[q] = a.p[q].blk0;
  const GnFwdProb& p = a.p[find_prob(blk0, a.nprob)];
  const int lane = threadIdx.x & 63, wave = threadIdx.x >> 6;
  const int K = p.K;
  const int rows = R == 1 ? 1 : p.rows;
  const int i = (int(blockIdx.x) - p.blk0) * (kFT / 64) + wave;
  const int ic = i < p.N ? i : p.N - 1;
  float4 w[KI];
#pragma unroll
  for (int u = 0; u < KI; ++u) {
    const int j = 4 * lane + 256 * u;
    w[u] = w4<BF>(p.W, p.Wh, int64_t(ic) * K + (j < K ? j : 0));
  }
  const bool ln = p.gam != nullptr;
  const float* gp = ln ? p.gam : p.x;
  const float* bp = ln ? p.bet : p.x;
  float xv[kPer], gv[kPer], bv[kPer];
#pragma unroll
  for (int u = 0; u < kPer; ++u) {
    const int j = int(threadIdx.x) + 256 * u, jc = j < K ? j : 0;
    xv[u] = p.x[jc];
    gv[u] = gp[jc];
    bv[u] = bp[jc];
  }
  float acc[R];
#pragma unroll
  for (int r = 0; r < R; ++r) {
    acc[r] = 0.f;
    if (r >= rows) continue;
    if (r > 0) {
      __syncthreads();
#pragma unroll
      for (int u = 0; u < kPer; ++u) {
        const int j = int(threadIdx.x) + 256 * u;
        xv[u] = p.x[int64_t(r) * K + (j < K ? j : 0)];
      }
    }
#pragma unroll
    for (int u = 0; u < kPer; ++u)
      if (int(threadIdx.x) + 256 * u >= K) xv[u] = 0.f;
    if (ln) {
      float mean, rstd;
      row_stats(xv, K, p.eps, scratch, mean, rstd);
#pragma unroll
      for (int u = 0; u < kPer; ++u) {
        const int j = int(threadIdx.x) + 256 * u;
        h[j] = j < K ? fmaxf(fmaf((xv[u] - mean) * rstd, gv[u], bv[u]), 0.f) : 0.f;
      }
    } else {
#pragma unroll
      for (int u = 0; u < kPer; ++u) h[int(threadIdx.x) + 256 * u] = xv[u];
    }
    __syncthreads();
#pragma unroll
    for (int u = 0; u < KI; ++u) {
      const int j = 4 * lane + 256 * u;
      if (j < kMaxK) {
        const float4 hv = *reinterpret_cast<const float4*>(h + j);
        acc[r] = fmaf(w[u].x, hv.x, fmaf(w[u].y, hv.y, fmaf(w[u].z, hv.z, fmaf(w[u].w, hv.w, acc[r]))));
      }
    }
  }
#pragma unroll
  for (int r = 0; r < R; ++r) {
    if (r >= rows) continue;
    const float v = wave_sum(acc[r]);
    if (lane == 0 && i < p.N)
      p.y[int64_t(r) * p.N + i] = v + (p.b ? p.b[i] : 0.f) + (p.res ? p.res[int64_t(r) * p.N + i] : 0.f);
  }
}

int launch_fwd(GnFwdArgs& a, hipStream_t st) {
  int blocks = 0, kmax = 0;
  for (int q = 0; q < a.nprob; ++q) {
    a.p[q].blk0 = blocks;
    blocks += (a.p[q].N + 3) / 4;
    kmax = a.p[q].K > kmax ? a.p[q].K : kmax;
  }
  for (int q = a.nprob; q < kMaxProb; ++q) a.p[q].blk0 = blocks;
  bool bf = true;
  for (int q = 0; q < a.nprob; ++q) bf = bf && a.p[q].Wh != nullptr;
  const int rows = a.p[0].rows;
  auto go = [&](auto k32, auto k16, auto m32, auto m16) {
    const auto kern = rows > 1 ? (bf ? m16 : m32) : (bf ? k16 : k32);
    hipLaunchKernelGGL(kern, dim3(blocks), dim3(kFT), 0, st, a);
  };
  constexpr int RM = kMaxRows;
  if (kmax <= 256)
    go(&gnode_fwd_kernel<1, false, 1>, &gnode_fwd_kernel<1, true, 1>, &gnode_fwd_kernel<1, false, RM>,
       &gnode_fwd_kernel<1, true, RM>);
  else if (kmax <= 1024)
    go(&gnode_fwd_kernel<4, false, 1>, &gnode_fwd_kernel<4, true, 1>, &gnode_fwd_kernel<4, false, RM>,
       &gnode_fwd_kernel<4, true, RM>);
  else if (kmax <= 1280)
    go(&gnode_fwd_kernel<5, false, 1>, &gnode_fwd_kernel<5, true, 1>, &gnode_fwd_kernel<5, false, RM>,
       &gnode_fwd_kernel<5, true, RM>);
  else
    go(&gnode_fwd_kernel<8, false, 1>, &gnode_fwd_kernel<8, true, 1>, &gnode_fwd_kernel<8, false, RM>,
       &gnode_fwd_kernel<8, true, RM>);
  return launch_status("gasfm_gchain_fwd");
}

struct GnBwdProb {
  const float* dy;
  const float* x;
  const float* gam;
  const float* bet;
  const float* W;
  float* dW;
  float* db;
  float* dh;
  float* ws;
  uint32_t* cnt;
  int K, N, blk0, slabs, chunks;
  float eps;
  float* dgam;
  float* dbet;
  float* lnp;
  float* stats;
  int lnfin;
  const uint16_t* Wh;
  int rows;
};
struct GnPro {
  const float* gv[kMaxRaw];
  const float* lnp[kMaxRaw];
  const float* stats;
  const float* x;
  const float* dres;
  float* out;
  int nq, F, slabs;
};
struct GnBwdArgs {
  GnBwdProb p[kMaxProb];
  GnPro pro;
  int nprob;
};

__device__ __forceinline__ void st_sc1(float* p, float4 v) {
  uint64_t a, b;
  __builtin_memcpy(&a, &v.x, 8);
  __builtin_memcpy(&b, &v.z, 8);
  __hip_atomic_store(reinterpret_cast<uint64_t*>(p), a, __ATOMIC_RELAXED, __HIP_MEMORY_SCOPE_AGENT);
  __hip_atomic_store(reinterpret_cast<uint64_t*>(p) + 1, b, __ATOMIC_RELAXED, __HIP_MEMORY_SCOPE_AGENT);
}
__device__ __forceinline__ float ld_sc1(const float* p) {
  return __hip_atomic_load(p, __ATOMIC_RELAXED, __HIP_MEMORY_SCOPE_AGENT);
}

template <int RPT, bool BF, int R>
__global__ __launch_bounds__(kBT) void gnode_bwd_kernel(GnBwdArgs a) {
  static_assert(32 * RPT == kBT, "one dy row per thread");
  __shared__ float dys[R][32 * RPT];
  __shared__ float4 red[kBT];
  __shared__ float scratch[4 * 2 * kMaxRaw * R + 8];
  __shared__ uint32_t flag;
  int blk0[kMaxProb];
#pragma unroll
  for (int q = 0; q < kMaxProb; ++q) blk0[q] = a.p[q].blk0;
  const int pi = find_prob(blk0, a.nprob);
  const GnBwdProb& p = a.p[pi];
  const int rows = R == 1 ? 1 : p.rows;
  const int local = int(blockIdx.x) - p.blk0;
  const int slab = local % p.slabs, chunk = local / p.slabs;
  const int cl = threadIdx.x & 7, rl = threadIdx.x >> 3;
  const int K = p.K, N = p.N;
  const int col = slab * kSW + 4 * cl;
  const int row0 = chunk * 32 * RPT;
  const int nrow = row0 + int(threadIdx.x), nrc = nrow < N ? nrow : N - 1;
  const GnPro& pr = a.pro;
  const bool pro = pr.nq > 0;
  float dres[R], xr[R], gvr[R][kMaxRaw], lp[R * 2 * kMaxRaw], st0[R], st1[R], dyv[R];
#pragma unroll
  for (int r = 0; r < R; ++r) {
    dres[r] = xr[r] = st0[r] = st1[r] = dyv[r] = 0.f;
#pragma unroll
    for (int q = 0; q < kMaxRaw; ++q) {
      gvr[r][q] = 0.f;
      lp[(r * kMaxRaw + q) * 2] = lp[(r * kMaxRaw + q) * 2 + 1] = 0.f;
    }
    if (r >= rows) continue;
    if (pro) {
      const int64_t ro = int64_t(r) * pr.F;
      dres[r] = pr.dres ? pr.dres[ro + nrc] : 0.f;
      xr[r] = pr.x[ro + nrc];
      st0[r] = pr.stats[2 * r];
      st1[r] = pr.stats[2 * r + 1];
      const int tc = int(threadIdx.x) < pr.slabs ? int(threadIdx.x) : 0;
#pragma unroll
      for (int q = 0; q < kMaxRaw; ++q) {
        const bool on = q < pr.nq;
        gvr[r][q] = on ? pr.gv[q][ro + nrc] : 0.f;
        const int64_t lo = (int64_t(r) * pr.slabs + tc) * 2;
        lp[(r * kMaxRaw + q) * 2] = on ? pr.lnp[q][lo] : 0.f;
        lp[(r * kMaxRaw + q) * 2 + 1] = on ? pr.lnp[q][lo + 1] : 0.f;
      }
    } else {
      dyv[r] = p.dy[int64_t(r) * N + nrc];
    }
  }
  float4 w[RPT];
#pragma unroll
  for (int k = 0; k < RPT; ++k) {
    const int n = row0 + rl + 32 * k;
    w[k] = w4<BF>(p.W, p.Wh, int64_t(n < N ? n : N - 1) * K + col);
  }
  float4 x4[R];
#pragma unroll
  for (int r = 0; r < R; ++r) x4[r] = *reinterpret_cast<const float4*>(p.x + int64_t(r < rows ? r : 0) * K + col);
  const bool ln = p.gam != nullptr;
  float4 g4 = x4[0], b4 = x4[0];
  float xv[kPer];
  if (ln) {
    g4 = *reinterpret_cast<const float4*>(p.gam + col);
    b4 = *reinterpret_cast<const float4*>(p.bet + col);
#pragma unroll
    for (int u = 0; u < kPer; ++u) {
      const int j = int(threadIdx.x) + 256 * u;
      xv[u] = p.x[j < K ? j : 0];
    }
#pragma unroll
    for (int u = 0; u < kPer; ++u)
      if (int(threadIdx.x) + 256 * u >= K) xv[u] = 0.f;
  }
  if (pro) {
    if (int(threadIdx.x) >= pr.slabs) {
#pragma unroll
      for (int k = 0; k < R * 2 * kMaxRaw; ++k) lp[k] = 0.f;
    }
    block_sums<R * 2 * kMaxRaw>(lp, scratch);
    const float invF = 1.f / pr.F;
#pragma unroll
    for (int r = 0; r < R; ++r) {
      if (r >= rows) continue;
      const float xh = (xr[r] - st0[r]) * st1[r];
      float d = dres[r];
#pragma unroll
      for (int q = 0; q < kMaxRaw; ++q)
        if (q < pr.nq)
          d += st1[r] * (gvr[r][q] - lp[(r * kMaxRaw + q) * 2] * invF - xh * lp[(r * kMaxRaw + q) * 2 + 1] * invF);
      dyv[r] = d;
      if (slab == 0 && pr.out && nrow < N) pr.out[int64_t(r) * pr.F + nrow] = d;
    }
  }
#pragma unroll
  for (int r = 0; r < R; ++r) dys[r][threadIdx.x] = (nrow < N && r < rows) ? dyv[r] : 0.f;
  float4 h4[R], xh4[R];
  float mean[R], rstd[R];
#pragma unroll
  for (int r = 0; r < R; ++r) {
    h4[r] = xh4[r] = x4[r];
    mean[r] = rstd[r] = 0.f;
    if (ln && r < rows) {
      if (r > 0) {
#pragma unroll
        for (int u = 0; u < kPer; ++u) {
          const int j = int(threadIdx.x) + 256 * u;
          xv[u] = j < K ? p.x[int64_t(r) * K + j] : 0.f;
        }
      }
      __syncthreads();
      row_stats(xv, K, p.eps, scratch, mean[r], rstd[r]);
      const float4 xx = x4[r];
      xh4[r] = make_float4((xx.x - mean[r]) * rstd[r], (xx.y - mean[r]) * rstd[r], (xx.z - mean[r]) * rstd[r],
                           (xx.w - mean[r]) * rstd[r]);
      h4[r] = make_float4(fmaxf(fmaf(xh4[r].x, g4.x, b4.x), 0.f), fmaxf(fmaf(xh4[r].y, g4.y, b4.y), 0.f),
                          fmaxf(fmaf(xh4[r].z, g4.z, b4.z), 0.f), fmaxf(fmaf(xh4[r].w, g4.w, b4.w), 0.f));
    }
  }
  __syncthreads();
  auto store_dw = [&]() {
#pragma unroll
    for (int k = 0; k < RPT; ++k) {
      const int n = row0 + rl + 32 * k;
      float4 v = make_float4(0.f, 0.f, 0.f, 0.f);
#pragma unroll
      for (int r = 0; r < R; ++r) {
        if (r >= rows) continue;
        const float d = dys[r][rl + 32 * k];
        v.x = fmaf(d, h4[r].x, v.x);
        v.y = fmaf(d, h4[r].y, v.y);
        v.z = fmaf(d, h4[r].z, v.z);
        v.w = fmaf(d, h4[r].w, v.w);
      }
      if (n < N) *reinterpret_cast<float4*>(p.dW + int64_t(n) * K + col) = v;
    }
    if (p.db && slab == 0 && nrow < N) {
      float v = 0.f;
#pragma unroll
      for (int r = 0; r < R; ++r)
        if (r < rows) v += dys[r][threadIdx.x];
      p.db[nrow] = v;
    }
  };
  float4 tot[R];
#pragma unroll
  for (int r = 0; r < R; ++r) {
    tot[r] = make_float4(0.f, 0.f, 0.f, 0.f);
    if (r >= rows) continue;
    float4 sv = make_float4(0.f, 0.f, 0.f, 0.f);
#pragma unroll
    for (int k = 0; k < RPT; ++k) {
      const float d = dys[r][rl + 32 * k];
      sv.x = fmaf(d, w[k].x, sv.x);
      sv.y = fmaf(d, w[k].y, sv.y);
      sv.z = fmaf(d, w[k].z, sv.z);
      sv.w = fmaf(d, w[k].w, sv.w);
    }
    if (r > 0) __syncthreads();
    red[threadIdx.x] = sv;
    __syncthreads();
    if (threadIdx.x < 8) {
#pragma unroll 8
      for (int l = 0; l < 32; ++l) {
        const float4 v = red[l * 8 + threadIdx.x];
        tot[r].x += v.x;
        tot[r].y += v.y;
        tot[r].z += v.z;
        tot[r].w += v.w;
      }
    }
  }
  if (p.chunks > 1) {
    if (threadIdx.x < 8) {
#pragma unroll
      for (int r = 0; r < R; ++r)
        if (r < rows) st_sc1(p.ws + (int64_t(chunk) * rows + r) * K + col, tot[r]);
    }
    asm volatile("s_waitcnt vmcnt(0)" ::: "memory");
    __syncthreads();
    if (threadIdx.x == 0) {
      const uint32_t t = __hip_atomic_fetch_add(p.cnt + slab, 1u, __ATOMIC_RELAXED, __HIP_MEMORY_SCOPE_AGENT);
      flag = t == uint32_t(p.chunks - 1) ? 1u : 0u;
    }
    __syncthreads();
    if (flag == 0u) {
      store_dw();
      return;
    }
    __builtin_amdgcn_fence(__ATOMIC_ACQUIRE, "wavefront");
    if (threadIdx.x < 8) {
      constexpr int MAXC = 16;
#pragma unroll
      for (int r = 0; r < R; ++r) {
        if (r >= rows) continue;
        float4 v[MAXC];
#pragma unroll
        for (int ch = 0; ch < MAXC; ++ch) {
          const float* q = p.ws + (int64_t(ch < p.chunks ? ch : 0) * rows + r) * K + col;
          v[ch] = make_float4(ld_sc1(q), ld_sc1(q + 1), ld_sc1(q + 2), ld_sc1(q + 3));
        }
        tot[r] = make_float4(0.f, 0.f, 0.f, 0.f);
#pragma unroll
        for (int ch = 0; ch < MAXC; ++ch)
          if (ch < p.chunks) {
            tot[r].x += v[ch].x;
            tot[r].y += v[ch].y;
            tot[r].z += v[ch].z;
            tot[r].w += v[ch].w;
          }
      }
    }
    if (threadIdx.x == 0) __hip_atomic_store(p.cnt + slab, 0u, __ATOMIC_RELAXED, __HIP_MEMORY_SCOPE_AGENT);
  }
  if (threadIdx.x < 8) {
    if (p.lnfin) {
      const float gg[4] = {g4.x, g4.y, g4.z, g4.w};
      const float bb[4] = {b4.x, b4.y, b4.z, b4.w};
      float dg[4] = {0.f, 0.f, 0.f, 0.f}, db[4] = {0.f, 0.f, 0.f, 0.f};
#pragma unroll
      for (int r = 0; r < R; ++r) {
        if (r >= rows) continue;
        const float t4[4] = {tot[r].x, tot[r].y, tot[r].z, tot[r].w};
        const float xh[4] = {xh4[r].x, xh4[r].y, xh4[r].z, xh4[r].w};
        float d[4], gv[4], s1 = 0.f, s2 = 0.f;
#pragma unroll
        for (int k = 0; k < 4; ++k) {
          d[k] = fmaf(xh[k], gg[k], bb[k]) > 0.f ? t4[k] : 0.f;
          gv[k] = d[k] * gg[k];
          s1 += gv[k];
          s2 = fmaf(gv[k], xh[k], s2);
          dg[k] = fmaf(d[k], xh[k], dg[k]);
          db[k] += d[k];
        }
        *reinterpret_cast<float4*>(p.dh + int64_t(r) * K + col) = make_float4(gv[0], gv[1], gv[2], gv[3]);
#pragma unroll
        for (int o = 1; o < 8; o <<= 1) {
          s1 += __shfl_xor(s1, o);
          s2 += __shfl_xor(s2, o);
        }
        if (threadIdx.x == 0) {
          p.lnp[(int64_t(r) * p.slabs + slab) * 2] = s1;
          p.lnp[(int64_t(r) * p.slabs + slab) * 2 + 1] = s2;
          if (slab == 0 && p.stats) {
            p.stats[2 * r] = mean[r];
            p.stats[2 * r + 1] = rstd[r];
          }
        }
      }
      *reinterpret_cast<float4*>(p.dgam + col) = make_float4(dg[0], dg[1], dg[2], dg[3]);
      *reinterpret_cast<float4*>(p.dbet + col) = make_float4(db[0], db[1], db[2], db[3]);
    } else {
#pragma unroll
      for (int r = 0; r < R; ++r)
        if (r < rows) *reinterpret_cast<float4*>(p.dh + int64_t(r) * K + col) = tot[r];
    }
  }
  store_dw();
}

template <int RPT, bool BF, int R>
__global__ __launch_bounds__(kBT) void gnode_bwd_rows_kernel(GnBwdArgs a) {
  static_assert(32 * RPT == kBT, "one dy row per thread");
  __shared__ float dys[R][32 * RPT];
  __shared__ float4 red[R][kBT];
  __shared__ float4 tots[R][8];
  __shared__ float scratch[4 * R + 8];
  __shared__ uint32_t flag;
  int blk0[kMaxProb];
#pragma unroll
  for (int q = 0; q < kMaxProb; ++q) blk0[q] = a.p[q].blk0;
  const int pi = find_prob(blk0, a.nprob);
  const GnBwdProb& p = a.p[pi];
  const int rows = p.rows;
  const int local = int(blockIdx.x) - p.blk0;
  const int slab = local % p.slabs, chunk = local / p.slabs;
  const int cl = threadIdx.x & 7, rl = threadIdx.x >> 3, lane = threadIdx.x & 63;
  const int K = p.K, N = p.N;
  const int col = slab * kSW + 4 * cl;
  const int row0 = chunk * 32 * RPT;
  const int nrow = row0 + int(threadIdx.x), nrc = nrow < N ? nrow : N - 1;
  const GnPro& pr = a.pro;
  const bool pro = pr.nq > 0;
  float4 w[RPT];
#pragma unroll
  for (int k = 0; k < RPT; ++k) {
    const int n = row0 + rl + 32 * k;
    w[k] = w4<BF>(p.W, p.Wh, int64_t(n < N ? n : N - 1) * K + col);
  }
  const float invF = pro ? 1.f / pr.F : 0.f;
  for (int r = 0; r < rows; ++r) {
    float d;
    if (pro) {
      const int64_t ro = int64_t(r) * pr.F;
      const int tl = lane < pr.slabs ? lane : 0;
      float gq[kMaxRaw], l1[kMaxRaw], l2[kMaxRaw];
#pragma unroll
      for (int q = 0; q < kMaxRaw; ++q) {
        const bool on = q < pr.nq;
        gq[q] = on ? pr.gv[q][ro + nrc] : 0.f;
        const int64_t lo = (int64_t(r) * pr.slabs + tl) * 2;
        l1[q] = on && lane < pr.slabs ? pr.lnp[q][lo] : 0.f;
        l2[q] = on && lane < pr.slabs ? pr.lnp[q][lo + 1] : 0.f;
      }
      d = pr.dres ? pr.dres[ro + nrc] : 0.f;
      const float m0 = pr.stats[2 * r], r0 = pr.stats[2 * r + 1];
      const float xh = (pr.x[ro + nrc] - m0) * r0;
#pragma unroll
      for (int q = 0; q < kMaxRaw; ++q) {
        const float s1 = wave_sum(l1[q]), s2 = wave_sum(l2[q]);
        if (q < pr.nq) d += r0 * (gq[q] - s1 * invF - xh * s2 * invF);
      }
      if (slab == 0 && pr.out && nrow < N) pr.out[ro + nrow] = d;
    } else {
      d = p.dy[int64_t(r) * N + nrc];
    }
    dys[r][threadIdx.x] = nrow < N ? d : 0.f;
  }
  const bool ln = p.gam != nullptr;
  float4 g4 = make_float4(0.f, 0.f, 0.f, 0.f), b4 = g4;
  float mean[R], rstd[R];
#pragma unroll
  for (int r = 0; r < R; ++r) mean[r] = rstd[r] = 0.f;
  if (ln) {
    g4 = *reinterpret_cast<const float4*>(p.gam + col);
    b4 = *reinterpret_cast<const float4*>(p.bet + col);
    float sx[R];
#pragma unroll
    for (int r = 0; r < R; ++r) {
      sx[r] = 0.f;
      if (r < rows)
#pragma unroll
        for (int u = 0; u < kPer; ++u) {
          const int j = int(threadIdx.x) + 256 * u;
          sx[r] += j < K ? p.x[int64_t(r) * K + j] : 0.f;
        }
    }
    block_sums<R>(sx, scratch);
#pragma unroll
    for (int r = 0; r < R; ++r) mean[r] = sx[r] / K;
    float sq[R];
#pragma unroll
    for (int r = 0; r < R; ++r) {
      sq[r] = 0.f;
      if (r < rows)
#pragma unroll
        for (int u = 0; u < kPer; ++u) {
          const int j = int(threadIdx.x) + 256 * u;
          const float dd = j < K ? p.x[int64_t(r) * K + j] - mean[r] : 0.f;
          sq[r] = fmaf(dd, dd, sq[r]);
        }
    }
    block_sums<R>(sq, scratch);
#pragma unroll
    for (int r = 0; r < R; ++r) rstd[r] = rsq_normal(sq[r] / K + p.eps);
  }
  __syncthreads();
#pragma unroll
  for (int r = 0; r < R; ++r) {
    if (r >= rows) continue;
    float4 sv = make_float4(0.f, 0.f, 0.f, 0.f);
#pragma unroll
    for (int k = 0; k < RPT; ++k) {
      const float d = dys[r][rl + 32 * k];
      sv.x = fmaf(d, w[k].x, sv.x);
      sv.y = fmaf(d, w[k].y, sv.y);
      sv.z = fmaf(d, w[k].z, sv.z);
      sv.w = fmaf(d, w[k].w, sv.w);
    }
    red[r][threadIdx.x] = sv;
  }
  __syncthreads();
  const int tr = threadIdx.x >> 3;
  const bool rowlane = int(threadIdx.x) < 8 * rows;
  if (rowlane) {
    float4 t = make_float4(0.f, 0.f, 0.f, 0.f);
#pragma unroll 8
    for (int l = 0; l < 32; ++l) {
      const float4 v = red[tr][l * 8 + cl];
      t.x += v.x;
      t.y += v.y;
      t.z += v.z;
      t.w += v.w;
    }
    tots[tr][cl] = t;
  }
  auto hrow = [&](int r, float4& xh, float4& h) {
    const float4 x4 = *reinterpret_cast<const float4*>(p.x + int64_t(r) * K + col);
    if (!ln) {
      xh = h = x4;
      return;
    }
    xh = make_float4((x4.x - mean[r]) * rstd[r], (x4.y - mean[r]) * rstd[r], (x4.z - mean[r]) * rstd[r],
                     (x4.w - mean[r]) * rstd[r]);
    h = make_float4(fmaxf(fmaf(xh.x, g4.x, b4.x), 0.f), fmaxf(fmaf(xh.y, g4.y, b4.y), 0.f),
                    fmaxf(fmaf(xh.z, g4.z, b4.z), 0.f), fmaxf(fmaf(xh.w, g4.w, b4.w), 0.f));
  };
  auto store_dw = [&]() {
    float4 hs[R];
#pragma unroll
    for (int r = 0; r < R; ++r) {
      float4 xh;
      hs[r] = make_float4(0.f, 0.f, 0.f, 0.f);
      if (r < rows) hrow(r, xh, hs[r]);
    }
#pragma unroll
    for (int k = 0; k < RPT; ++k) {
      const int n = row0 + rl + 32 * k;
      float4 v = make_float4(0.f, 0.f, 0.f, 0.f);
#pragma unroll
      for (int r = 0; r < R; ++r) {
        if (r >= rows) continue;
        const float d = dys[r][rl + 32 * k];
        v.x = fmaf(d, hs[r].x, v.x);
        v.y = fmaf(d, hs[r].y, v.y);
        v.z = fmaf(d, hs[r].z, v.z);
        v.w = fmaf(d, hs[r].w, v.w);
      }
      if (n < N) *reinterpret_cast<float4*>(p.dW + int64_t(n) * K + col) = v;
    }
    if (p.db && slab == 0 && nrow < N) {
      float v = 0.f;
      for (int r = 0; r < rows; ++r) v += dys[r][threadIdx.x];
      p.db[nrow] = v;
    }
  };
  if (p.chunks > 1) {
    if (rowlane) st_sc1(p.ws + (int64_t(chunk) * rows + tr) * K + col, tots[tr][cl]);
    asm volatile("s_waitcnt vmcnt(0)" ::: "memory");
    __syncthreads();
    if (threadIdx.x == 0) {
      const uint32_t t = __hip_atomic_fetch_add(p.cnt + slab, 1u, __ATOMIC_RELAXED, __HIP_MEMORY_SCOPE_AGENT);
      flag = t == uint32_t(p.chunks - 1) ? 1u : 0u;
    }
    __syncthreads();
    if (flag == 0u) {
      store_dw();
      return;
    }
    __builtin_amdgcn_fence(__ATOMIC_ACQUIRE, "wavefront");
    if (rowlane) {
      constexpr int MAXC = 16;
      float4 v[MAXC];
#pragma unroll
      for (int ch = 0; ch < MAXC; ++ch) {
        const float* q = p.ws + (int64_t(ch < p.chunks ? ch : 0) * rows + tr) * K + col;
        v[ch] = make_float4(ld_sc1(q), ld_sc1(q + 1), ld_sc1(q + 2), ld_sc1(q + 3));
      }
      float4 t = make_float4(0.f, 0.f, 0.f, 0.f);
#pragma unroll
      for (int ch = 0; ch < MAXC; ++ch)
        if (ch < p.chunks) {
          t.x += v[ch].x;
          t.y += v[ch].y;
          t.z += v[ch].z;
          t.w += v[ch].w;
        }
      tots[tr][cl] = t;
    }
    if (threadIdx.x == 0) __hip_atomic_store(p.cnt + slab, 0u, __ATOMIC_RELAXED, __HIP_MEMORY_SCOPE_AGENT);
  }
  if (p.lnfin) {
    float4 dgr = make_float4(0.f, 0.f, 0.f, 0.f), dbr = dgr;
    if (rowlane) {
      float4 xh4, h4;
      hrow(tr, xh4, h4);
      const float4 tt = tots[tr][cl];
      const float t4[4] = {tt.x, tt.y, tt.z, tt.w};
      const float xh[4] = {xh4.x, xh4.y, xh4.z, xh4.w};
      const float gg[4] = {g4.x, g4.y, g4.z, g4.w};
      const float bb[4] = {b4.x, b4.y, b4.z, b4.w};
      float d[4], gv[4], s1 = 0.f, s2 = 0.f;
#pragma unroll
      for (int k = 0; k < 4; ++k) {
        d[k] = fmaf(xh[k], gg[k], bb[k]) > 0.f ? t4[k] : 0.f;
        gv[k] = d[k] * gg[k];
        s1 += gv[k];
        s2 = fmaf(gv[k], xh[k], s2);
      }
      dgr = make_float4(d[0] * xh[0], d[1] * xh[1], d[2] * xh[2], d[3] * xh[3]);
      dbr = make_float4(d[0], d[1], d[2], d[3]);
      *reinterpret_cast<float4*>(p.dh + int64_t(tr) * K + col) = make_float4(gv[0], gv[1], gv[2], gv[3]);
#pragma unroll
      for (int o = 1; o < 8; o <<= 1) {
        s1 += __shfl_xor(s1, o);
        s2 += __shfl_xor(s2, o);
      }
      if (cl == 0) {
        p.lnp[(int64_t(tr) * p.slabs + slab) * 2] = s1;
        p.lnp[(int64_t(tr) * p.slabs + slab) * 2 + 1] = s2;
        if (slab == 0 && p.stats) {
          p.stats[2 * tr] = mean[tr];
          p.stats[2 * tr + 1] = rstd[tr];
        }
      }
    }
    __syncthreads();
    if (rowlane) {
      red[tr][cl] = dgr;
      red[tr][8 + cl] = dbr;
    }
    __syncthreads();
    if (threadIdx.x < 8) {
      float4 dg = make_float4(0.f, 0.f, 0.f, 0.f), db = dg;
      for (int r = 0; r < rows; ++r) {
        const float4 a4 = red[r][threadIdx.x], b4v = red[r][8 + threadIdx.x];
        dg.x += a4.x;
        dg.y += a4.y;
        dg.z += a4.z;
        dg.w += a4.w;
        db.x += b4v.x;
        db.y += b4v.y;
        db.z += b4v.z;
        db.w += b4v.w;
      }
      *reinterpret_cast<float4*>(p.dgam + col) = dg;
      *reinterpret_cast<float4*>(p.dbet + col) = db;
    }
  } else if (rowlane) {
    *reinterpret_cast<float4*>(p.dh + int64_t(tr) * K + col) = tots[tr][cl];
  }
  store_dw();
}

constexpr int kRPT = 8;

int chunks_of(int N) { return (N + 32 * kRPT - 1) / (32 * kRPT); }

int launch_bwd(GnBwdArgs& a, int rows, float*& ws, uint32_t*& cnt, hipStream_t st, const char* where) {
  int blocks = 0;
  for (int q = 0; q < a.nprob; ++q) {
    GnBwdProb& p = a.p[q];
    p.blk0 = blocks;
    p.slabs = p.K / kSW;
    p.chunks = chunks_of(p.N);
    p.ws = ws;
    p.cnt = cnt;
    p.rows = rows;
    ws += int64_t(p.chunks) * rows * p.K;
    cnt += p.slabs;
    blocks += p.slabs * p.chunks;
  }
  for (int q = a.nprob; q < kMaxProb; ++q) a.p[q].blk0 = blocks;
  bool bf = true;
  for (int q = 0; q < a.nprob; ++q) bf = bf && a.p[q].Wh != nullptr;
  const auto kern = rows > 1 ? (bf ? &gnode_bwd_rows_kernel<kRPT, true, kMaxRows>
                                    : &gnode_bwd_rows_kernel<kRPT, false, kMaxRows>)
                             : (bf ? &gnode_bwd_kernel<kRPT, true, 1> : &gnode_bwd_kernel<kRPT, false, 1>);
  hipLaunchKernelGGL(kern, dim3(blocks), dim3(kBT), 0, st, a);
  return launch_status(where);
}

int rows_of(const gasfm_gchain* c) { return c->rows > 1 ? c->rows : 1; }

bool hub_on(const gasfm_gchain* c) { return c->NB > 0; }

}
}

using namespace gasfm;

static int gchain_check(const gasfm_gchain* c) {
  GASFM_REQUIRE(c, "gasfm_gchain: null parameters");
  GASFM_REQUIRE(c->G > 0 && c->G <= kMaxK && c->G % kSW == 0 && c->Kc > 0 && c->Kc <= kMaxK && c->Kc % kSW == 0 &&
                    c->NA > 0 && c->NA <= kMaxK,
                "gasfm_gchain: G=%d Kc=%d NA=%d (multiples of %d, <= %d)", c->G, c->Kc, c->NA, kSW, kMaxK);
  GASFM_REQUIRE(c->W1 && c->b1 && c->gM && c->bM && c->W2 && c->b2 && c->gA && c->bA && c->WA,
                "gasfm_gchain: null weight");
  if (c->NB > 0) {
    GASFM_REQUIRE(c->NB <= kMaxK && c->NB % kSW == 0 && c->NC > 0 && c->NC <= kMaxK && c->NC % kSW == 0 &&
                      c->ND > 0 && c->ND <= kMaxK && c->NE > 0 && c->NE <= kMaxK,
                  "gasfm_gchain: NB=%d NC=%d ND=%d NE=%d", c->NB, c->NC, c->ND, c->NE);
    GASFM_REQUIRE(c->gB && c->bB && c->WB && c->bWB && c->gC && c->bC && c->WC && c->bWC && c->WD && c->bD && c->WE &&
                      c->bE,
                  "gasfm_gchain: null hub weight");
  }
  GASFM_REQUIRE(c->rows >= 0 && c->rows <= kMaxRows, "gasfm_gchain: rows=%d (<= %d)", c->rows, kMaxRows);
  const void* ws[] = {c->W1, c->W2, c->WA, c->WB, c->WC, c->WD, c->WE};
  for (const void* p : ws) GASFM_REQUIRE(!p || aligned16(p), "gasfm_gchain: weights must be 16-byte aligned");
  const void* wh[] = {c->W1h, c->W2h, c->WAh, c->WBh, c->WCh, c->WDh, c->WEh};
  for (const void* p : wh)
    GASFM_REQUIRE(!p || reinterpret_cast<uintptr_t>(p) % 8 == 0, "gasfm_gchain: bf16 shadows must be 8-byte aligned");
  return GASFM_OK;
}

extern "C" int64_t gasfm_gchain_scratch_floats(const gasfm_gchain* c) {
  if (!c) return 0;
  const int64_t R = rows_of(c);
  const int64_t vec = int64_t(c->NB) + c->NC + 4 * int64_t(c->G);
  const int64_t lnp = 4 * 2 * int64_t(c->G / kSW) + 8;
  const int64_t l1 = int64_t(chunks_of(c->ND)) * c->NB + int64_t(chunks_of(c->NE)) * c->NC;
  const int64_t l2 = int64_t(chunks_of(c->NA) + chunks_of(c->NB) + chunks_of(c->NC)) * c->G;
  const int64_t l3 = int64_t(chunks_of(c->G)) * c->G;
  const int64_t l4 = int64_t(chunks_of(c->G)) * c->Kc;
  return R * (vec + lnp + l1 + l2 + l3 + l4 + c->G) + 64;
}

extern "C" int32_t gasfm_gchain_counters(const gasfm_gchain* c) {
  if (!c) return 0;
  return (c->NB + c->NC + 4 * c->G + c->Kc) / kSW + 8;
}

extern "C" int gasfm_gchain_fwd(const gasfm_gchain* c, const float* xcat, const float* prev, float* x1, float* g,
                                float* sg, float* xv, float* xp, float* xrv, float* xrp, void* stream) {
  const int s0 = gchain_check(c);
  if (s0 != GASFM_OK) return s0;
  GASFM_REQUIRE(xcat && x1 && g && sg && (!hub_on(c) || (xv && xp && xrv && xrp)), "gasfm_gchain_fwd: null output");
  hipStream_t st = reinterpret_cast<hipStream_t>(stream);
  const int R = rows_of(c);
  GnFwdArgs a{};
  a.nprob = 1;
  a.p[0] = GnFwdProb{xcat, nullptr, nullptr, c->W1, c->b1, prev, x1, c->Kc, c->G, 0, 0.f, c->W1h, R};
  int s = launch_fwd(a, st);
  if (s != GASFM_OK) return s;
  a.p[0] = GnFwdProb{x1, c->gM, c->bM, c->W2, c->b2, x1, g, c->G, c->G, 0, c->eps_m, c->W2h, R};
  s = launch_fwd(a, st);
  if (s != GASFM_OK) return s;
  a.p[0] = GnFwdProb{g, c->gA, c->bA, c->WA, nullptr, nullptr, sg, c->G, c->NA, 0, c->eps_h, c->WAh, R};
  if (hub_on(c)) {
    a.nprob = 3;
    a.p[1] = GnFwdProb{g, c->gB, c->bB, c->WB, c->bWB, nullptr, xv, c->G, c->NB, 0, c->eps_h, c->WBh, R};
    a.p[2] = GnFwdProb{g, c->gC, c->bC, c->WC, c->bWC, nullptr, xp, c->G, c->NC, 0, c->eps_h, c->WCh, R};
  }
  s = launch_fwd(a, st);
  if (s != GASFM_OK || !hub_on(c)) return s;
  a.nprob = 2;
  a.p[0] = GnFwdProb{xv, nullptr, nullptr, c->WD, c->bD, nullptr, xrv, c->NB, c->ND, 0, 0.f, c->WDh, R};
  a.p[1] = GnFwdProb{xp, nullptr, nullptr, c->WE, c->bE, nullptr, xrp, c->NC, c->NE, 0, 0.f, c->WEh, R};
  return launch_fwd(a, st);
}

extern "C" int gasfm_gchain_bwd(const gasfm_gchain* c, const float* xcat, const float* x1, const float* g,
                                const float* xv, const float* xp, const float* dskip, const float* dsg,
                                const float* dxrv, const float* dxrp, float* dxcat, float* dprev,
                                const gasfm_gchain_grads* d, float* scratch, uint32_t* counters, void* stream) {
  const int s0 = gchain_check(c);
  if (s0 != GASFM_OK) return s0;
  GASFM_REQUIRE(d && xcat && x1 && g && dsg && dxcat && scratch && counters, "gasfm_gchain_bwd: null pointer");
  GASFM_REQUIRE(d->dW1 && d->db1 && d->dgM && d->dbM && d->dW2 && d->db2 && d->dgA && d->dbA && d->dWA,
                "gasfm_gchain_bwd: null gradient");
  const bool hub = hub_on(c);
  if (hub)
    GASFM_REQUIRE(xv && xp && dxrv && dxrp && d->dgB && d->dbB && d->dWB && d->dbWB && d->dgC && d->dbC && d->dWC &&
                      d->dbWC && d->dWD && d->dbD && d->dWE && d->dbE,
                  "gasfm_gchain_bwd: null hub pointer");
  hipStream_t st = reinterpret_cast<hipStream_t>(stream);
  const int slabsG = c->G / kSW;
  const int R = rows_of(c);
  float* dhD = scratch;
  float* dhE = dhD + int64_t(R) * c->NB;
  float* gvA = dhE + int64_t(R) * c->NC;
  float* gvB = gvA + int64_t(R) * c->G;
  float* gvC = gvB + int64_t(R) * c->G;
  float* gv2 = gvC + int64_t(R) * c->G;
  float* lnA = gv2 + int64_t(R) * c->G;
  float* lnB = lnA + 2 * R * slabsG;
  float* lnC = lnB + 2 * R * slabsG;
  float* ln2 = lnC + 2 * R * slabsG;
  float* stg = ln2 + 2 * R * slabsG;
  float* st1 = stg + 2 * R;
  float* dgr = st1 + 2 * R + 4;
  float* ws = dgr + int64_t(R) * c->G;
  uint32_t* cnt = counters;
  int s;
  if (hub) {
    GnBwdArgs a{};
    a.nprob = 2;
    a.p[0] = GnBwdProb{dxrv, xv, nullptr, nullptr, c->WD, d->dWD, d->dbD, dhD};
    a.p[0].K = c->NB, a.p[0].N = c->ND, a.p[0].Wh = c->WDh;
    a.p[1] = GnBwdProb{dxrp, xp, nullptr, nullptr, c->WE, d->dWE, d->dbE, dhE};
    a.p[1].K = c->NC, a.p[1].N = c->NE, a.p[1].Wh = c->WEh;
    s = launch_bwd(a, R, ws, cnt, st, "gasfm_gchain_bwd(lin_r)");
    if (s != GASFM_OK) return s;
  }
  {
    GnBwdArgs a{};
    a.nprob = hub ? 3 : 1;
    auto lnprob = [&](const float* dy, const float* gam, const float* bet, const float* W, const uint16_t* Wh,
                      float* dW, float* db, int N, float* gv, float* dgam, float* dbet, float* lnp, float* stats) {
      GnBwdProb p{dy, g, gam, bet, W, dW, db, gv};
      p.K = c->G, p.N = N, p.eps = c->eps_h, p.Wh = Wh;
      p.dgam = dgam, p.dbet = dbet, p.lnp = lnp, p.stats = stats, p.lnfin = 1;
      return p;
    };
    a.p[0] = lnprob(dsg, c->gA, c->bA, c->WA, c->WAh, d->dWA, nullptr, c->NA, gvA, d->dgA, d->dbA, lnA, stg);
    if (hub) {
      a.p[1] = lnprob(dhD, c->gB, c->bB, c->WB, c->WBh, d->dWB, d->dbWB, c->NB, gvB, d->dgB, d->dbB, lnB, nullptr);
      a.p[2] = lnprob(dhE, c->gC, c->bC, c->WC, c->WCh, d->dWC, d->dbWC, c->NC, gvC, d->dgC, d->dbC, lnC, nullptr);
    }
    s = launch_bwd(a, R, ws, cnt, st, "gasfm_gchain_bwd(hub)");
    if (s != GASFM_OK) return s;
  }
  {
    GnBwdArgs a{};
    a.nprob = 1;
    GnBwdProb& p = a.p[0];
    p = GnBwdProb{nullptr, x1, c->gM, c->bM, c->W2, d->dW2, d->db2, gv2};
    p.K = c->G, p.N = c->G, p.eps = c->eps_m, p.Wh = c->W2h;
    p.dgam = d->dgM, p.dbet = d->dbM, p.lnp = ln2, p.stats = st1, p.lnfin = 1;
    GnPro& pr = a.pro;
    pr.nq = hub ? 3 : 1;
    pr.gv[0] = gvA, pr.lnp[0] = lnA;
    pr.gv[1] = gvB, pr.lnp[1] = lnB;
    pr.gv[2] = gvC, pr.lnp[2] = lnC;
    pr.stats = stg, pr.x = g, pr.dres = dskip, pr.out = R > 1 ? dgr : nullptr, pr.F = c->G, pr.slabs = slabsG;
    s = launch_bwd(a, R, ws, cnt, st, "gasfm_gchain_bwd(mlp)");
    if (s != GASFM_OK) return s;
  }
  GnBwdArgs a{};
  a.nprob = 1;
  a.p[0] = GnBwdProb{nullptr, xcat, nullptr, nullptr, c->W1, d->dW1, d->db1, dxcat};
  a.p[0].K = c->Kc, a.p[0].N = c->G, a.p[0].Wh = c->W1h;
  GnPro& pr = a.pro;
  pr.nq = 1;
  pr.gv[0] = gv2, pr.lnp[0] = ln2;
  pr.stats = st1, pr.x = x1, pr.dres = R > 1 ? dgr : d->db2, pr.out = dprev, pr.F = c->G, pr.slabs = slabsG;
  return launch_bwd(a, R, ws, cnt, st, "gasfm_gchain_bwd(proj)");
}
```

Baseline: 144.4 million edges/s.

## Fuse global-chain forward/backward levels into one persistent kernel with grid barriers

Replaces the sequence of per-level global-chain forward and backward launches with a single persistent kernel. Levels are separated by sharded atomic arrive counters, and intermediates are passed through coherent (agent-scope atomic) loads and stores. W rows are loaded into registers once per block, and the bias-gradient store is moved earlier. This targets launch overhead and inter-kernel gaps in this small-row global path. In exchange it adds spin-wait barriers, coherent-memory traffic, a residency requirement for the grid, and a fallback to multi-launch when fusion is not possible.

```diff
diff --git a/gasfm_amd/_native.py b/gasfm_amd/_native.py
--- a/gasfm_amd/_native.py
+++ b/gasfm_amd/_native.py
@@ -1283,9 +1283,9 @@
 
 
 def gchain_fwd(c, xcat, prev, x1, g, sg, xv, xp, xrv, xrp):
-    st = lib().gasfm_gchain_fwd(ctypes.addressof(c), _p(xcat), _p(prev), _p(x1), _p(g), _p(sg), _p(xv), _p(xp),
-                                _p(xrv), _p(xrp), _stream(g))
-    check(st, "gasfm_gchain_fwd")
+    from .gchain import _binding as gcf
+    st = gcf.fwd(c, (xcat, prev, x1, g, sg, xv, xp, xrv, xrp), g.device, _stream(g))
+    check(st, "gasfm_gchain_fwd_fused")
 
 
 def gchain_bwd(c, xcat, x1, g, xv, xp, dskip, dsg, dxrv, dxrp, dxcat, dprev, grads):
@@ -1297,10 +1297,9 @@
     L = lib()
     ws = torch.empty(int(L.gasfm_gchain_scratch_floats(ctypes.addressof(c))), dtype=torch.float32, device=g.device)
     cnt = _counters(g.device, L.gasfm_gchain_counters(ctypes.addressof(c)))
-    st = L.gasfm_gchain_bwd(ctypes.addressof(c), _p(xcat), _p(x1), _p(g), _p(xv), _p(xp), _p(dskip), _p(dsg),
-                            _p(dxrv), _p(dxrp), _p(dxcat), _p(dprev), ctypes.addressof(d), _p(ws), _p(cnt),
-                            _stream(g))
-    check(st, "gasfm_gchain_bwd")
+    from .gchain import _binding as gcf
+    st = gcf.bwd(c, (xcat, x1, g, xv, xp, dskip, dsg, dxrv, dxrp, dxcat, dprev), d, ws, cnt, g.device, _stream(g))
+    check(st, "gasfm_gchain_bwd_fused")
 
 
 _GattProb = _abi.structs["gasfm_gatt_prob"]
diff --git a/gasfm_amd/build.py b/gasfm_amd/build.py
--- a/gasfm_amd/build.py
+++ b/gasfm_amd/build.py
@@ -8,6 +8,7 @@
 LIB = os.path.join(HERE, "libgasfm.so")
 HEADER = os.path.join(HERE, "..", "include", "gasfm.h")
 DEPTH_HEAD_HEADER = os.path.join(HERE, "..", "include", "gasfm_depth_head.h")
+GCHAIN_FUSED_HEADER = os.path.join(HERE, "..", "include", "gasfm_gchain_fused.h")
 ARCH = os.environ.get("GASFM_OFFLOAD_ARCH", "gfx950")
 
 
@@ -26,7 +27,7 @@
     if not os.path.exists(LIB):
         return True
     t = os.path.getmtime(LIB)
-    deps = sources() + glob.glob(os.path.join(CSRC, "*.hpp")) + [HEADER, DEPTH_HEAD_HEADER]
+    deps = sources() + glob.glob(os.path.join(CSRC, "*.hpp")) + [HEADER, DEPTH_HEAD_HEADER, GCHAIN_FUSED_HEADER]
     return any(os.path.getmtime(p) > t for p in deps if os.path.exists(p))
 
 
diff --git a/gasfm_amd/csrc/global_chain.hip b/gasfm_amd/csrc/global_chain.hip
--- a/gasfm_amd/csrc/global_chain.hip
+++ b/gasfm_amd/csrc/global_chain.hip
@@ -1,8 +1,11 @@
 #include <hip/hip_runtime.h>
 
+#include <atomic>
 #include <cstdint>
+#include <cstdlib>
 
 #include "common.hpp"
+#include "../../include/gasfm_gchain_fused.h"
 
 namespace gasfm {
 namespace {
@@ -74,10 +77,39 @@
 }
 
 template <int NP>
-__device__ __forceinline__ int find_prob(const int (&blk0)[NP], int nprob) {
+__device__ __forceinline__ int find_prob(const int (&blk0)[NP], int nprob, int blk) {
   int pi = 0;
-  while (pi + 1 < nprob && int(blockIdx.x) >= blk0[pi + 1]) ++pi;
+  while (pi + 1 < nprob && blk >= blk0[pi + 1]) ++pi;
   return pi;
+}
+
+__device__ __forceinline__ void st_sc1(float* p, float4 v) {
+  uint64_t a, b;
+  __builtin_memcpy(&a, &v.x, 8);
+  __builtin_memcpy(&b, &v.z, 8);
+  __hip_atomic_store(reinterpret_cast<uint64_t*>(p), a, __ATOMIC_RELAXED, __HIP_MEMORY_SCOPE_AGENT);
+  __hip_atomic_store(reinterpret_cast<uint64_t*>(p) + 1, b, __ATOMIC_RELAXED, __HIP_MEMORY_SCOPE_AGENT);
+}
+__device__ __forceinline__ float ld_sc1(const float* p) {
+  return __hip_atomic_load(p, __ATOMIC_RELAXED, __HIP_MEMORY_SCOPE_AGENT);
+}
+template <bool CO>
+__device__ __forceinline__ float ldv(const float* p) {
+  return CO ? ld_sc1(p) : *p;
+}
+template <bool CO>
+__device__ __forceinline__ void stv(float* p, float v) {
+  if (CO)
+    __hip_atomic_store(p, v, __ATOMIC_RELAXED, __HIP_MEMORY_SCOPE_AGENT);
+  else
+    *p = v;
+}
+template <bool CO>
+__device__ __forceinline__ void stv4(float* p, float4 v) {
+  if (CO)
+    st_sc1(p, v);
+  else
+    *reinterpret_cast<float4*>(p) = v;
 }
 
 struct GnFwdProb {
@@ -98,25 +130,35 @@
   int nprob;
 };
 
-template <int KI, bool BF, int R>
-__global__ __launch_bounds__(kFT) void gnode_fwd_kernel(GnFwdArgs a) {
-  __shared__ __attribute__((aligned(16))) float h[kMaxK];
-  __shared__ float scratch[8];
+template <int KI, bool BF, int NW>
+__device__ __forceinline__ void fwd_load_w(const GnFwdArgs& a, int blk, float4 (&w)[NW], int ki = KI) {
+  static_assert(KI <= NW, "W row registers");
   int blk0[kMaxProb];
 #pragma unroll
   for (int q = 0; q < kMaxProb; ++q) blk0[q] = a.p[q].blk0;
-  const GnFwdProb& p = a.p[find_prob(blk0, a.nprob)];
+  const GnFwdProb& p = a.p[find_prob(blk0, a.nprob, blk)];
+  const int lane = threadIdx.x & 63, wave = threadIdx.x >> 6;
+  const int K = p.K;
+  const int i = (blk - p.blk0) * (kFT / 64) + wave;
+  const int ic = i < p.N ? i : p.N - 1;
+#pragma unroll
+  for (int u = 0; u < KI; ++u) {
+    const int j = 4 * lane + 256 * u;
+    if (u < ki) w[u] = w4<BF>(p.W, p.Wh, int64_t(ic) * K + (j < K ? j : 0));
+  }
+}
+
+template <int KI, bool BF, int R, bool CO, int NW>
+__device__ __forceinline__ void fwd_body(const GnFwdArgs& a, int blk, const float4 (&w)[NW], float* h,
+                                         float* scratch, int ki = KI) {
+  int blk0[kMaxProb];
+#pragma unroll
+  for (int q = 0; q < kMaxProb; ++q) blk0[q] = a.p[q].blk0;
+  const GnFwdProb& p = a.p[find_prob(blk0, a.nprob, blk)];
   const int lane = threadIdx.x & 63, wave = threadIdx.x >> 6;
   const int K = p.K;
   const int rows = R == 1 ? 1 : p.rows;
-  const int i = (int(blockIdx.x) - p.blk0) * (kFT / 64) + wave;
-  const int ic = i < p.N ? i : p.N - 1;
-  float4 w[KI];
-#pragma unroll
-  for (int u = 0; u < KI; ++u) {
-    const int j = 4 * lane + 256 * u;
-    w[u] = w4<BF>(p.W, p.Wh, int64_t(ic) * K + (j < K ? j : 0));
-  }
+  const int i = (blk - p.blk0) * (kFT / 64) + wave;
   const bool ln = p.gam != nullptr;
   const float* gp = ln ? p.gam : p.x;
   const float* bp = ln ? p.bet : p.x;
@@ -124,7 +166,7 @@
 #pragma unroll
   for (int u = 0; u < kPer; ++u) {
     const int j = int(threadIdx.x) + 256 * u, jc = j < K ? j : 0;
-    xv[u] = p.x[jc];
+    xv[u] = ldv<CO>(p.x + jc);
     gv[u] = gp[jc];
     bv[u] = bp[jc];
   }
@@ -138,7 +180,7 @@
 #pragma unroll
       for (int u = 0; u < kPer; ++u) {
         const int j = int(threadIdx.x) + 256 * u;
-        xv[u] = p.x[int64_t(r) * K + (j < K ? j : 0)];
+        xv[u] = ldv<CO>(p.x + int64_t(r) * K + (j < K ? j : 0));
       }
     }
 #pragma unroll
@@ -160,7 +202,7 @@
 #pragma unroll
     for (int u = 0; u < KI; ++u) {
       const int j = 4 * lane + 256 * u;
-      if (j < kMaxK) {
+      if (j < kMaxK && u < ki) {
         const float4 hv = *reinterpret_cast<const float4*>(h + j);
         acc[r] = fmaf(w[u].x, hv.x, fmaf(w[u].y, hv.y, fmaf(w[u].z, hv.z, fmaf(w[u].w, hv.w, acc[r]))));
       }
@@ -171,20 +213,42 @@
     if (r >= rows) continue;
     const float v = wave_sum(acc[r]);
     if (lane == 0 && i < p.N)
-      p.y[int64_t(r) * p.N + i] = v + (p.b ? p.b[i] : 0.f) + (p.res ? p.res[int64_t(r) * p.N + i] : 0.f);
-  }
-}
-
-int launch_fwd(GnFwdArgs& a, hipStream_t st) {
-  int blocks = 0, kmax = 0;
+      stv<CO>(p.y + int64_t(r) * p.N + i,
+              v + (p.b ? p.b[i] : 0.f) + (p.res ? ldv<CO>(p.res + int64_t(r) * p.N + i) : 0.f));
+  }
+}
+
+template <int KI, bool BF, int R>
+__global__ __launch_bounds__(kFT) void gnode_fwd_kernel(GnFwdArgs a) {
+  __shared__ __attribute__((aligned(16))) float h[kMaxK];
+  __shared__ float scratch[8];
+  float4 w[KI];
+  fwd_load_w<KI, BF>(a, int(blockIdx.x), w);
+  fwd_body<KI, BF, R, false>(a, int(blockIdx.x), w, h, scratch);
+}
+
+int fill_fwd(GnFwdArgs& a, int& kmax) {
+  int blocks = 0;
+  kmax = 0;
   for (int q = 0; q < a.nprob; ++q) {
     a.p[q].blk0 = blocks;
     blocks += (a.p[q].N + 3) / 4;
     kmax = a.p[q].K > kmax ? a.p[q].K : kmax;
   }
   for (int q = a.nprob; q < kMaxProb; ++q) a.p[q].blk0 = blocks;
+  return blocks;
+}
+
+bool all_bf(const GnFwdArgs& a) {
   bool bf = true;
   for (int q = 0; q < a.nprob; ++q) bf = bf && a.p[q].Wh != nullptr;
+  return bf;
+}
+
+int launch_fwd(GnFwdArgs& a, hipStream_t st) {
+  int kmax = 0;
+  const int blocks = fill_fwd(a, kmax);
+  const bool bf = all_bf(a);
   const int rows = a.p[0].rows;
   auto go = [&](auto k32, auto k16, auto m32, auto m16) {
     const auto kern = rows > 1 ? (bf ? m16 : m32) : (bf ? k16 : k32);
@@ -242,31 +306,54 @@
   int nprob;
 };
 
-__device__ __forceinline__ void st_sc1(float* p, float4 v) {
-  uint64_t a, b;
-  __builtin_memcpy(&a, &v.x, 8);
-  __builtin_memcpy(&b, &v.z, 8);
-  __hip_atomic_store(reinterpret_cast<uint64_t*>(p), a, __ATOMIC_RELAXED, __HIP_MEMORY_SCOPE_AGENT);
-  __hip_atomic_store(reinterpret_cast<uint64_t*>(p) + 1, b, __ATOMIC_RELAXED, __HIP_MEMORY_SCOPE_AGENT);
-}
-__device__ __forceinline__ float ld_sc1(const float* p) {
-  return __hip_atomic_load(p, __ATOMIC_RELAXED, __HIP_MEMORY_SCOPE_AGENT);
-}
-
-template <int RPT, bool BF, int R>
-__global__ __launch_bounds__(kBT) void gnode_bwd_kernel(GnBwdArgs a) {
+template <int R>
+struct BwdShared {
+  float dys[R][kBT];
+  float4 red[kBT];
+  float scratch[4 * 2 * kMaxRaw * R + 8];
+  uint32_t flag;
+};
+
+constexpr int kShards = 8;
+constexpr int kShardStride = 32;
+__device__ __forceinline__ void grid_arrive(uint32_t* c) {
+  __hip_atomic_fetch_add(c + kShardStride * (int(blockIdx.x) % kShards), 1u, __ATOMIC_RELAXED,
+                         __HIP_MEMORY_SCOPE_AGENT);
+}
+
+template <int RPT, bool BF>
+__device__ __forceinline__ void bwd_load_w(const GnBwdArgs& a, int blk, float4 (&w)[RPT]) {
+  int blk0[kMaxProb];
+#pragma unroll
+  for (int q = 0; q < kMaxProb; ++q) blk0[q] = a.p[q].blk0;
+  const GnBwdProb& p = a.p[find_prob(blk0, a.nprob, blk)];
+  const int local = blk - p.blk0;
+  const int slab = local % p.slabs, chunk = local / p.slabs;
+  const int cl = threadIdx.x & 7, rl = threadIdx.x >> 3;
+  const int col = slab * kSW + 4 * cl;
+  const int row0 = chunk * 32 * RPT;
+#pragma unroll
+  for (int k = 0; k < RPT; ++k) {
+    const int n = row0 + rl + 32 * k;
+    w[k] = w4<BF>(p.W, p.Wh, int64_t(n < p.N ? n : p.N - 1) * p.K + col);
+  }
+}
+
+template <int RPT, bool BF, int R, bool CO>
+__device__ __forceinline__ void bwd_body(const GnBwdArgs& a, int blk, const float4 (&w)[RPT], BwdShared<R>& sh,
+                                         uint32_t* arrive) {
   static_assert(32 * RPT == kBT, "one dy row per thread");
-  __shared__ float dys[R][32 * RPT];
-  __shared__ float4 red[kBT];
-  __shared__ float scratch[4 * 2 * kMaxRaw * R + 8];
-  __shared__ uint32_t flag;
+  auto& dys = sh.dys;
+  auto& red = sh.red;
+  float* scratch = sh.scratch;
+  uint32_t& flag = sh.flag;
   int blk0[kMaxProb];
 #pragma unroll
   for (int q = 0; q < kMaxProb; ++q) blk0[q] = a.p[q].blk0;
-  const int pi = find_prob(blk0, a.nprob);
+  const int pi = find_prob(blk0, a.nprob, blk);
   const GnBwdProb& p = a.p[pi];
   const int rows = R == 1 ? 1 : p.rows;
-  const int local = int(blockIdx.x) - p.blk0;
+  const int local = blk - p.blk0;
   const int slab = local % p.slabs, chunk = local / p.slabs;
   const int cl = threadIdx.x & 7, rl = threadIdx.x >> 3;
   const int K = p.K, N = p.N;
@@ -287,28 +374,22 @@
     if (r >= rows) continue;
     if (pro) {
       const int64_t ro = int64_t(r) * pr.F;
-      dres[r] = pr.dres ? pr.dres[ro + nrc] : 0.f;
+      dres[r] = pr.dres ? ldv<CO>(pr.dres + ro + nrc) : 0.f;
       xr[r] = pr.x[ro + nrc];
-      st0[r] = pr.stats[2 * r];
-      st1[r] = pr.stats[2 * r + 1];
+      st0[r] = ldv<CO>(pr.stats + 2 * r);
+      st1[r] = ldv<CO>(pr.stats + 2 * r + 1);
       const int tc = int(threadIdx.x) < pr.slabs ? int(threadIdx.x) : 0;
 #pragma unroll
       for (int q = 0; q < kMaxRaw; ++q) {
         const bool on = q < pr.nq;
-        gvr[r][q] = on ? pr.gv[q][ro + nrc] : 0.f;
+        gvr[r][q] = on ? ldv<CO>(pr.gv[q] + ro + nrc) : 0.f;
         const int64_t lo = (int64_t(r) * pr.slabs + tc) * 2;
-        lp[(r * kMaxRaw + q) * 2] = on ? pr.lnp[q][lo] : 0.f;
-        lp[(r * kMaxRaw + q) * 2 + 1] = on ? pr.lnp[q][lo + 1] : 0.f;
+        lp[(r * kMaxRaw + q) * 2] = on ? ldv<CO>(pr.lnp[q] + lo) : 0.f;
+        lp[(r * kMaxRaw + q) * 2 + 1] = on ? ldv<CO>(pr.lnp[q] + lo + 1) : 0.f;
       }
     } else {
-      dyv[r] = p.dy[int64_t(r) * N + nrc];
-    }
-  }
-  float4 w[RPT];
-#pragma unroll
-  for (int k = 0; k < RPT; ++k) {
-    const int n = row0 + rl + 32 * k;
-    w[k] = w4<BF>(p.W, p.Wh, int64_t(n < N ? n : N - 1) * K + col);
+      dyv[r] = ldv<CO>(p.dy + int64_t(r) * N + nrc);
+    }
   }
   float4 x4[R];
 #pragma unroll
@@ -345,11 +426,18 @@
         if (q < pr.nq)
           d += st1[r] * (gvr[r][q] - lp[(r * kMaxRaw + q) * 2] * invF - xh * lp[(r * kMaxRaw + q) * 2 + 1] * invF);
       dyv[r] = d;
-      if (slab == 0 && pr.out && nrow < N) pr.out[int64_t(r) * pr.F + nrow] = d;
+      if (slab == 0 && pr.out && nrow < N) stv<CO>(pr.out + int64_t(r) * pr.F + nrow, d);
     }
   }
 #pragma unroll
   for (int r = 0; r < R; ++r) dys[r][threadIdx.x] = (nrow < N && r < rows) ? dyv[r] : 0.f;
+  if (p.db && slab == 0 && nrow < N) {
+    float v = 0.f;
+#pragma unroll
+    for (int r = 0; r < R; ++r)
+      if (r < rows) v += dyv[r];
+    stv<CO>(p.db + nrow, v);
+  }
   float4 h4[R], xh4[R];
   float mean[R], rstd[R];
 #pragma unroll
@@ -389,13 +477,6 @@
         v.w = fmaf(d, h4[r].w, v.w);
       }
       if (n < N) *reinterpret_cast<float4*>(p.dW + int64_t(n) * K + col) = v;
-    }
-    if (p.db && slab == 0 && nrow < N) {
-      float v = 0.f;
-#pragma unroll
-      for (int r = 0; r < R; ++r)
-        if (r < rows) v += dys[r][threadIdx.x];
-      p.db[nrow] = v;
     }
   };
   float4 tot[R];
@@ -440,6 +521,7 @@
     }
     __syncthreads();
     if (flag == 0u) {
+      if (CO && threadIdx.x == 0) grid_arrive(arrive);
       store_dw();
       return;
     }
@@ -488,18 +570,18 @@
           dg[k] = fmaf(d[k], xh[k], dg[k]);
           db[k] += d[k];
         }
-        *reinterpret_cast<float4*>(p.dh + int64_t(r) * K + col) = make_float4(gv[0], gv[1], gv[2], gv[3]);
+        stv4<CO>(p.dh + int64_t(r) * K + col, make_float4(gv[0], gv[1], gv[2], gv[3]));
 #pragma unroll
         for (int o = 1; o < 8; o <<= 1) {
           s1 += __shfl_xor(s1, o);
           s2 += __shfl_xor(s2, o);
         }
         if (threadIdx.x == 0) {
-          p.lnp[(int64_t(r) * p.slabs + slab) * 2] = s1;
-          p.lnp[(int64_t(r) * p.slabs + slab) * 2 + 1] = s2;
+          stv<CO>(p.lnp + (int64_t(r) * p.slabs + slab) * 2, s1);
+          stv<CO>(p.lnp + (int64_t(r) * p.slabs + slab) * 2 + 1, s2);
           if (slab == 0 && p.stats) {
-            p.stats[2 * r] = mean[r];
-            p.stats[2 * r + 1] = rstd[r];
+            stv<CO>(p.stats + 2 * r, mean[r]);
+            stv<CO>(p.stats + 2 * r + 1, rstd[r]);
           }
         }
       }
@@ -508,10 +590,23 @@
     } else {
 #pragma unroll
       for (int r = 0; r < R; ++r)
-        if (r < rows) *reinterpret_cast<float4*>(p.dh + int64_t(r) * K + col) = tot[r];
-    }
+        if (r < rows) stv4<CO>(p.dh + int64_t(r) * K + col, tot[r]);
+    }
+  }
+  if (CO) {
+    asm volatile("s_waitcnt vmcnt(0)" ::: "memory");
+    __syncthreads();
+    if (threadIdx.x == 0) grid_arrive(arrive);
   }
   store_dw();
+}
+
+template <int RPT, bool BF, int R>
+__global__ __launch_bounds__(kBT) void gnode_bwd_kernel(GnBwdArgs a) {
+  __shared__ BwdShared<R> sh;
+  float4 w[RPT];
+  bwd_load_w<RPT, BF>(a, int(blockIdx.x), w);
+  bwd_body<RPT, BF, R, false>(a, int(blockIdx.x), w, sh, nullptr);
 }
 
 template <int RPT, bool BF, int R>
@@ -525,7 +620,7 @@
   int blk0[kMaxProb];
 #pragma unroll
   for (int q = 0; q < kMaxProb; ++q) blk0[q] = a.p[q].blk0;
-  const int pi = find_prob(blk0, a.nprob);
+  const int pi = find_prob(blk0, a.nprob, int(blockIdx.x));
   const GnBwdProb& p = a.p[pi];
   const int rows = p.rows;
   const int local = int(blockIdx.x) - p.blk0;
@@ -782,7 +877,7 @@
 
 int chunks_of(int N) { return (N + 32 * kRPT - 1) / (32 * kRPT); }
 
-int launch_bwd(GnBwdArgs& a, int rows, float*& ws, uint32_t*& cnt, hipStream_t st, const char* where) {
+int fill_bwd(GnBwdArgs& a, int rows, float*& ws, uint32_t*& cnt) {
   int blocks = 0;
   for (int q = 0; q < a.nprob; ++q) {
     GnBwdProb& p = a.p[q];
@@ -797,13 +892,148 @@
     blocks += p.slabs * p.chunks;
   }
   for (int q = a.nprob; q < kMaxProb; ++q) a.p[q].blk0 = blocks;
+  return blocks;
+}
+
+bool all_bf(const GnBwdArgs& a) {
   bool bf = true;
   for (int q = 0; q < a.nprob; ++q) bf = bf && a.p[q].Wh != nullptr;
+  return bf;
+}
+
+int launch_bwd(const GnBwdArgs& a, int blocks, int rows, hipStream_t st, const char* where) {
+  const bool bf = all_bf(a);
   const auto kern = rows > 1 ? (bf ? &gnode_bwd_rows_kernel<kRPT, true, kMaxRows>
                                     : &gnode_bwd_rows_kernel<kRPT, false, kMaxRows>)
                              : (bf ? &gnode_bwd_kernel<kRPT, true, 1> : &gnode_bwd_kernel<kRPT, false, 1>);
   hipLaunchKernelGGL(kern, dim3(blocks), dim3(kBT), 0, st, a);
   return launch_status(where);
+}
+
+constexpr int kLevels = 4;
+constexpr int kMaxPolls = 1 << 15;
+constexpr int kDoneWord = kShardStride * kShards * kLevels;
+static_assert(kDoneWord + 1 <= GASFM_GCHAIN_SYNC_WORDS, "sync words");
+
+__device__ __forceinline__ uint32_t* level_counter(uint32_t* sync, int L) {
+  return sync + kShardStride * kShards * L;
+}
+
+__device__ __forceinline__ bool grid_wait(uint32_t* c, uint32_t expect, uint32_t* status, uint32_t code,
+                                          uint32_t* okf) {
+  if (threadIdx.x < 64) {
+    const int lane = threadIdx.x;
+    bool ok = false;
+    for (int it = 0; it < kMaxPolls; ++it) {
+      uint32_t v = lane < kShards ? __hip_atomic_load(c + kShardStride * lane, __ATOMIC_RELAXED,
+                                                      __HIP_MEMORY_SCOPE_AGENT)
+                                  : 0u;
+#pragma unroll
+      for (int o = 1; o < kShards; o <<= 1) v += __shfl_xor(v, o);
+      ok = __shfl(v, 0) == expect;
+      if (ok) break;
+      __builtin_amdgcn_s_sleep(10);
+    }
+    if (lane == 0) {
+      *okf = ok ? 1u : 0u;
+      if (!ok) __hip_atomic_store(status, code, __ATOMIC_RELAXED, __HIP_MEMORY_SCOPE_AGENT);
+    }
+  }
+  __syncthreads();
+  const bool ok = *okf != 0u;
+  __builtin_amdgcn_fence(__ATOMIC_ACQUIRE, "wavefront");
+  return ok;
+}
+
+__device__ __forceinline__ void grid_leave(uint32_t* sync) {
+  if (threadIdx.x == 0) {
+    asm volatile("s_waitcnt vmcnt(0)" ::: "memory");
+    const uint32_t t = __hip_atomic_fetch_add(sync + kDoneWord, 1u, __ATOMIC_RELAXED, __HIP_MEMORY_SCOPE_AGENT);
+    if (t == gridDim.x - 1) {
+      for (int k = 0; k < kLevels * kShards; ++k)
+        __hip_atomic_store(sync + kShardStride * k, 0u, __ATOMIC_RELAXED, __HIP_MEMORY_SCOPE_AGENT);
+      __hip_atomic_store(sync + kDoneWord, 0u, __ATOMIC_RELAXED, __HIP_MEMORY_SCOPE_AGENT);
+    }
+  }
+}
+
+struct GcFwdArgs {
+  GnFwdArgs lv[kLevels];
+  int blocks[kLevels];
+  int ki[kLevels];
+  int nlev;
+  uint32_t* sync;
+  uint32_t* status;
+};
+
+template <bool BF>
+__global__ __launch_bounds__(kFT) void gchain_fwd_fused_kernel(GcFwdArgs a) {
+  __shared__ __attribute__((aligned(16))) float h[kMaxK];
+  __shared__ float scratch[8];
+  __shared__ uint32_t okf;
+  const int blk = int(blockIdx.x);
+  float4 w[8];
+  auto load = [&](const GnFwdArgs& lv, int ki) { fwd_load_w<8, BF>(lv, blk, w, ki); };
+  auto body = [&](const GnFwdArgs& lv, int ki) { fwd_body<8, BF, 1, true>(lv, blk, w, h, scratch, ki); };
+  bool live = true;
+  if (blk < a.blocks[0]) load(a.lv[0], a.ki[0]);
+#pragma unroll
+  for (int L = 0; L < kLevels; ++L) {
+    if (L < a.nlev && live && blk < a.blocks[L]) {
+      if (L > 0)
+        live = grid_wait(level_counter(a.sync, L - 1), uint32_t(a.blocks[L - 1]), a.status, uint32_t(L), &okf);
+      if (live) {
+        body(a.lv[L], a.ki[L]);
+        asm volatile("s_waitcnt vmcnt(0)" ::: "memory");
+        __syncthreads();
+        if (threadIdx.x == 0) grid_arrive(level_counter(a.sync, L));
+      }
+    }
+    if (L + 1 < kLevels && L + 1 < a.nlev && live && blk < a.blocks[L + 1]) load(a.lv[L + 1], a.ki[L + 1]);
+  }
+  grid_leave(a.sync);
+}
+
+struct GcBwdArgs {
+  GnBwdArgs lv[kLevels];
+  int blocks[kLevels];
+  int nlev;
+  uint32_t* sync;
+  uint32_t* status;
+};
+
+template <bool BF>
+__global__ __launch_bounds__(kBT) void gchain_bwd_fused_kernel(GcBwdArgs a) {
+  __shared__ BwdShared<1> sh;
+  __shared__ uint32_t okf;
+  const int blk = int(blockIdx.x);
+  float4 w[kRPT];
+  bool live = true;
+  if (blk < a.blocks[0]) bwd_load_w<kRPT, BF>(a.lv[0], blk, w);
+#pragma unroll
+  for (int L = 0; L < kLevels; ++L) {
+    if (L < a.nlev && live && blk < a.blocks[L]) {
+      if (L > 0)
+        live = grid_wait(level_counter(a.sync, L - 1), uint32_t(a.blocks[L - 1]), a.status, uint32_t(16 + L), &okf);
+      if (live) bwd_body<kRPT, BF, 1, true>(a.lv[L], blk, w, sh, level_counter(a.sync, L));
+    }
+    if (L + 1 < kLevels && L + 1 < a.nlev && live && blk < a.blocks[L + 1])
+      bwd_load_w<kRPT, BF>(a.lv[L + 1], blk, w);
+  }
+  grid_leave(a.sync);
+}
+
+std::atomic<int> g_fused{-1};
+std::atomic<long long> g_paths[2];
+
+bool fused_on() {
+  int v = g_fused.load(std::memory_order_relaxed);
+  if (v < 0) {
+    const char* e = std::getenv("GASFM_GCHAIN_FUSED");
+    v = e ? (std::atoi(e) != 0) : 0;
+    g_fused.store(v, std::memory_order_relaxed);
+  }
+  return v != 0;
 }
 
 int rows_of(const gasfm_gchain* c) { return c->rows > 1 ? c->rows : 1; }
@@ -856,39 +1086,89 @@
   return (c->NB + c->NC + 4 * c->G + c->Kc) / kSW + 8;
 }
 
-extern "C" int gasfm_gchain_fwd(const gasfm_gchain* c, const float* xcat, const float* prev, float* x1, float* g,
-                                float* sg, float* xv, float* xp, float* xrv, float* xrp, void* stream) {
+static int gchain_fwd_impl(const gasfm_gchain* c, const float* xcat, const float* prev, float* x1, float* g,
+                           float* sg, float* xv, float* xp, float* xrv, float* xrp, uint32_t* sync,
+                           uint32_t* status, void* stream) {
   const int s0 = gchain_check(c);
   if (s0 != GASFM_OK) return s0;
   GASFM_REQUIRE(xcat && x1 && g && sg && (!hub_on(c) || (xv && xp && xrv && xrp)), "gasfm_gchain_fwd: null output");
   hipStream_t st = reinterpret_cast<hipStream_t>(stream);
   const int R = rows_of(c);
-  GnFwdArgs a{};
-  a.nprob = 1;
-  a.p[0] = GnFwdProb{xcat, nullptr, nullptr, c->W1, c->b1, prev, x1, c->Kc, c->G, 0, 0.f, c->W1h, R};
-  int s = launch_fwd(a, st);
-  if (s != GASFM_OK) return s;
-  a.p[0] = GnFwdProb{x1, c->gM, c->bM, c->W2, c->b2, x1, g, c->G, c->G, 0, c->eps_m, c->W2h, R};
-  s = launch_fwd(a, st);
-  if (s != GASFM_OK) return s;
-  a.p[0] = GnFwdProb{g, c->gA, c->bA, c->WA, nullptr, nullptr, sg, c->G, c->NA, 0, c->eps_h, c->WAh, R};
+  GcFwdArgs f{};
+  f.nlev = hub_on(c) ? 4 : 3;
+  f.lv[0].nprob = 1;
+  f.lv[0].p[0] = GnFwdProb{xcat, nullptr, nullptr, c->W1, c->b1, prev, x1, c->Kc, c->G, 0, 0.f, c->W1h, R};
+  f.lv[1].nprob = 1;
+  f.lv[1].p[0] = GnFwdProb{x1, c->gM, c->bM, c->W2, c->b2, x1, g, c->G, c->G, 0, c->eps_m, c->W2h, R};
+  f.lv[2].nprob = 1;
+  f.lv[2].p[0] = GnFwdProb{g, c->gA, c->bA, c->WA, nullptr, nullptr, sg, c->G, c->NA, 0, c->eps_h, c->WAh, R};
   if (hub_on(c)) {
-    a.nprob = 3;
-    a.p[1] = GnFwdProb{g, c->gB, c->bB, c->WB, c->bWB, nullptr, xv, c->G, c->NB, 0, c->eps_h, c->WBh, R};
-    a.p[2] = GnFwdProb{g, c->gC, c->bC, c->WC, c->bWC, nullptr, xp, c->G, c->NC, 0, c->eps_h, c->WCh, R};
-  }
-  s = launch_fwd(a, st);
-  if (s != GASFM_OK || !hub_on(c)) return s;
-  a.nprob = 2;
-  a.p[0] = GnFwdProb{xv, nullptr, nullptr, c->WD, c->bD, nullptr, xrv, c->NB, c->ND, 0, 0.f, c->WDh, R};
-  a.p[1] = GnFwdProb{xp, nullptr, nullptr, c->WE, c->bE, nullptr, xrp, c->NC, c->NE, 0, 0.f, c->WEh, R};
-  return launch_fwd(a, st);
-}
-
-extern "C" int gasfm_gchain_bwd(const gasfm_gchain* c, const float* xcat, const float* x1, const float* g,
-                                const float* xv, const float* xp, const float* dskip, const float* dsg,
-                                const float* dxrv, const float* dxrp, float* dxcat, float* dprev,
-                                const gasfm_gchain_grads* d, float* scratch, uint32_t* counters, void* stream) {
+    f.lv[2].nprob = 3;
+    f.lv[2].p[1] = GnFwdProb{g, c->gB, c->bB, c->WB, c->bWB, nullptr, xv, c->G, c->NB, 0, c->eps_h, c->WBh, R};
+    f.lv[2].p[2] = GnFwdProb{g, c->gC, c->bC, c->WC, c->bWC, nullptr, xp, c->G, c->NC, 0, c->eps_h, c->WCh, R};
+    f.lv[3].nprob = 2;
+    f.lv[3].p[0] = GnFwdProb{xv, nullptr, nullptr, c->WD, c->bD, nullptr, xrv, c->NB, c->ND, 0, 0.f, c->WDh, R};
+    f.lv[3].p[1] = GnFwdProb{xp, nullptr, nullptr, c->WE, c->bE, nullptr, xrp, c->NC, c->NE, 0, 0.f, c->WEh, R};
+  }
+  bool fuse = sync && status && R == 1 && fused_on();
+  int grid = 0;
+  bool bf = false;
+  for (int L = 0; L < f.nlev && fuse; ++L) {
+    int kmax = 0;
+    f.blocks[L] = fill_fwd(f.lv[L], kmax);
+    f.ki[L] = kmax <= 256 ? 1 : kmax <= 1024 ? 4 : kmax <= 1280 ? 5 : 8;
+    const bool b = all_bf(f.lv[L]);
+    fuse = f.ki[L] != 1 && (L == 0 || b == bf);
+    bf = b;
+    grid = f.blocks[L] > grid ? f.blocks[L] : grid;
+  }
+  if (fuse) {
+    const auto kern = bf ? &gchain_fwd_fused_kernel<true> : &gchain_fwd_fused_kernel<false>;
+    fuse = grid <= resident_blocks(reinterpret_cast<const void*>(kern), kFT, 0);
+    if (fuse) {
+      f.sync = sync, f.status = status;
+      g_paths[0].fetch_add(1, std::memory_order_relaxed);
+      hipLaunchKernelGGL(kern, dim3(grid), dim3(kFT), 0, st, f);
+      return launch_status("gasfm_gchain_fwd(fused)");
+    }
+  }
+  g_paths[1].fetch_add(1, std::memory_order_relaxed);
+  for (int L = 0; L < f.nlev; ++L) {
+    const int s = launch_fwd(f.lv[L], st);
+    if (s != GASFM_OK) return s;
+  }
+  return GASFM_OK;
+}
+
+extern "C" int gasfm_gchain_fwd(const gasfm_gchain* c, const float* xcat, const float* prev, float* x1, float* g,
+                                float* sg, float* xv, float* xp, float* xrv, float* xrp, void* stream) {
+  return gchain_fwd_impl(c, xcat, prev, x1, g, sg, xv, xp, xrv, xrp, nullptr, nullptr, stream);
+}
+
+extern "C" int gasfm_gchain_fwd_fused(const void* cv, const float* xcat, const float* prev, float* x1,
+                                      float* g, float* sg, float* xv, float* xp, float* xrv, float* xrp,
+                                      uint32_t* sync, uint32_t* status, void* stream) {
+  GASFM_REQUIRE(sync && status, "gasfm_gchain_fwd_fused: null sync / status words");
+  const gasfm_gchain* c = static_cast<const gasfm_gchain*>(cv);
+  return gchain_fwd_impl(c, xcat, prev, x1, g, sg, xv, xp, xrv, xrp, sync, status, stream);
+}
+
+extern "C" int gasfm_gchain_fused_set(int32_t on) {
+  if (on >= 0) g_fused.store(on != 0, std::memory_order_relaxed);
+  return fused_on() ? 1 : 0;
+}
+
+extern "C" void gasfm_gchain_path_counts(int64_t* out) {
+  if (!out) return;
+  out[0] = g_paths[0].load(std::memory_order_relaxed);
+  out[1] = g_paths[1].load(std::memory_order_relaxed);
+}
+
+static int gchain_bwd_impl(const gasfm_gchain* c, const float* xcat, const float* x1, const float* g,
+                           const float* xv, const float* xp, const float* dskip, const float* dsg,
+                           const float* dxrv, const float* dxrp, float* dxcat, float* dprev,
+                           const gasfm_gchain_grads* d, float* scratch, uint32_t* counters, uint32_t* sync,
+                           uint32_t* status, void* stream) {
   const int s0 = gchain_check(c);
   if (s0 != GASFM_OK) return s0;
   GASFM_REQUIRE(d && xcat && x1 && g && dsg && dxcat && scratch && counters, "gasfm_gchain_bwd: null pointer");
@@ -917,19 +1197,21 @@
   float* dgr = st1 + 2 * R + 4;
   float* ws = dgr + int64_t(R) * c->G;
   uint32_t* cnt = counters;
-  int s;
+  GcBwdArgs f{};
+  const char* where[kLevels];
+  int nl = 0;
   if (hub) {
-    GnBwdArgs a{};
+    GnBwdArgs& a = f.lv[nl];
     a.nprob = 2;
     a.p[0] = GnBwdProb{dxrv, xv, nullptr, nullptr, c->WD, d->dWD, d->dbD, dhD};
     a.p[0].K = c->NB, a.p[0].N = c->ND, a.p[0].Wh = c->WDh;
     a.p[1] = GnBwdProb{dxrp, xp, nullptr, nullptr, c->WE, d->dWE, d->dbE, dhE};
     a.p[1].K = c->NC, a.p[1].N = c->NE, a.p[1].Wh = c->WEh;
-    s = launch_bwd(a, R, ws, cnt, st, "gasfm_gchain_bwd(lin_r)");
-    if (s != GASFM_OK) return s;
+    f.blocks[nl] = fill_bwd(a, R, ws, cnt);
+    where[nl++] = "gasfm_gchain_bwd(lin_r)";
   }
   {
-    GnBwdArgs a{};
+    GnBwdArgs& a = f.lv[nl];
     a.nprob = hub ? 3 : 1;
     auto lnprob = [&](const float* dy, const float* gam, const float* bet, const float* W, const uint16_t* Wh,
                       float* dW, float* db, int N, float* gv, float* dgam, float* dbet, float* lnp, float* stats) {
@@ -943,11 +1225,11 @@
       a.p[1] = lnprob(dhD, c->gB, c->bB, c->WB, c->WBh, d->dWB, d->dbWB, c->NB, gvB, d->dgB, d->dbB, lnB, nullptr);
       a.p[2] = lnprob(dhE, c->gC, c->bC, c->WC, c->WCh, d->dWC, d->dbWC, c->NC, gvC, d->dgC, d->dbC, lnC, nullptr);
     }
-    s = launch_bwd(a, R, ws, cnt, st, "gasfm_gchain_bwd(hub)");
-    if (s != GASFM_OK) return s;
+    f.blocks[nl] = fill_bwd(a, R, ws, cnt);
+    where[nl++] = "gasfm_gchain_bwd(hub)";
   }
   {
-    GnBwdArgs a{};
+    GnBwdArgs& a = f.lv[nl];
     a.nprob = 1;
     GnBwdProb& p = a.p[0];
     p = GnBwdProb{nullptr, x1, c->gM, c->bM, c->W2, d->dW2, d->db2, gv2};
@@ -959,10 +1241,10 @@
     pr.gv[1] = gvB, pr.lnp[1] = lnB;
     pr.gv[2] = gvC, pr.lnp[2] = lnC;
     pr.stats = stg, pr.x = g, pr.dres = dskip, pr.out = R > 1 ? dgr : nullptr, pr.F = c->G, pr.slabs = slabsG;
-    s = launch_bwd(a, R, ws, cnt, st, "gasfm_gchain_bwd(mlp)");
-    if (s != GASFM_OK) return s;
-  }
-  GnBwdArgs a{};
+    f.blocks[nl] = fill_bwd(a, R, ws, cnt);
+    where[nl++] = "gasfm_gchain_bwd(mlp)";
+  }
+  GnBwdArgs& a = f.lv[nl];
   a.nprob = 1;
   a.p[0] = GnBwdProb{nullptr, xcat, nullptr, nullptr, c->W1, d->dW1, d->db1, dxcat};
   a.p[0].K = c->Kc, a.p[0].N = c->G, a.p[0].Wh = c->W1h;
@@ -970,5 +1252,49 @@
   pr.nq = 1;
   pr.gv[0] = gv2, pr.lnp[0] = ln2;
   pr.stats = st1, pr.x = x1, pr.dres = R > 1 ? dgr : d->db2, pr.out = dprev, pr.F = c->G, pr.slabs = slabsG;
-  return launch_bwd(a, R, ws, cnt, st, "gasfm_gchain_bwd(proj)");
-}
+  f.blocks[nl] = fill_bwd(a, R, ws, cnt);
+  where[nl++] = "gasfm_gchain_bwd(proj)";
+  f.nlev = nl;
+  bool fuse = sync && status && R == 1 && fused_on();
+  const bool bf = all_bf(f.lv[0]);
+  int grid = 0;
+  for (int L = 0; L < nl; ++L) {
+    fuse = fuse && all_bf(f.lv[L]) == bf;
+    grid = f.blocks[L] > grid ? f.blocks[L] : grid;
+  }
+  if (fuse) {
+    const auto kern = bf ? &gchain_bwd_fused_kernel<true> : &gchain_bwd_fused_kernel<false>;
+    if (grid <= resident_blocks(reinterpret_cast<const void*>(kern), kBT, 0)) {
+      f.sync = sync, f.status = status;
+      g_paths[0].fetch_add(1, std::memory_order_relaxed);
+      hipLaunchKernelGGL(kern, dim3(grid), dim3(kBT), 0, st, f);
+      return launch_status("gasfm_gchain_bwd(fused)");
+    }
+  }
+  g_paths[1].fetch_add(1, std::memory_order_relaxed);
+  for (int L = 0; L < nl; ++L) {
+    const int s = launch_bwd(f.lv[L], f.blocks[L], R, st, where[L]);
+    if (s != GASFM_OK) return s;
+  }
+  return GASFM_OK;
+}
+
+extern "C" int gasfm_gchain_bwd(const gasfm_gchain* c, const float* xcat, const float* x1, const float* g,
+                                const float* xv, const float* xp, const float* dskip, const float* dsg,
+                                const float* dxrv, const float* dxrp, float* dxcat, float* dprev,
+                                const gasfm_gchain_grads* d, float* scratch, uint32_t* counters, void* stream) {
+  return gchain_bwd_impl(c, xcat, x1, g, xv, xp, dskip, dsg, dxrv, dxrp, dxcat, dprev, d, scratch, counters,
+                         nullptr, nullptr, stream);
+}
+
+extern "C" int gasfm_gchain_bwd_fused(const void* cv, const float* xcat, const float* x1, const float* g,
+                                      const float* xv, const float* xp, const float* dskip, const float* dsg,
+                                      const float* dxrv, const float* dxrp, float* dxcat, float* dprev,
+                                      const void* dv, float* scratch, uint32_t* counters, uint32_t* sync,
+                                      uint32_t* status, void* stream) {
+  GASFM_REQUIRE(sync && status, "gasfm_gchain_bwd_fused: null sync / status words");
+  const gasfm_gchain* c = static_cast<const gasfm_gchain*>(cv);
+  const gasfm_gchain_grads* d = static_cast<const gasfm_gchain_grads*>(dv);
+  return gchain_bwd_impl(c, xcat, x1, g, xv, xp, dskip, dsg, dxrv, dxrp, dxcat, dprev, d, scratch, counters, sync,
+                         status, stream);
+}
diff --git a/gasfm_amd/gchain/__init__.py b/gasfm_amd/gchain/__init__.py
--- /dev/null
+++ b/gasfm_amd/gchain/__init__.py
@@ -0,0 +1 @@
+from ._binding import fused_set, path_counts, status, status_word
diff --git a/gasfm_amd/gchain/_binding.py b/gasfm_amd/gchain/_binding.py
--- /dev/null
+++ b/gasfm_amd/gchain/_binding.py
@@ -0,0 +1,64 @@
+import ctypes
+
+import torch
+
+from .. import _abi, _native
+from ..build import GCHAIN_FUSED_HEADER
+
+
+with open(GCHAIN_FUSED_HEADER) as _f:
+    functions, constants, _ = _abi.parse(_f.read())
+SYNC_WORDS = constants["GASFM_GCHAIN_SYNC_WORDS"]
+_bound = None
+
+
+def lib_():
+    global _bound
+    L = _native.lib()
+    if _bound is not L:
+        for name, (res, args) in functions.items():
+            fn = getattr(L, name)
+            fn.restype = res
+            fn.argtypes = args
+        _bound = L
+    return L
+
+
+_STATUS = {}
+
+
+def status_word(device):
+    device = torch.device(device)
+    if device.index is None:
+        device = torch.device(device.type, torch.cuda.current_device())
+    t = _STATUS.get(device)
+    if t is None:
+        t = _STATUS[device] = torch.zeros(1, dtype=torch.int32, device=device)
+    return t
+
+
+def status(device):
+    return int(status_word(device).item())
+
+
+def fused_set(on):
+    return bool(lib_().gasfm_gchain_fused_set(-1 if on is None else int(bool(on))))
+
+
+def path_counts():
+    buf = (ctypes.c_int64 * 2)()
+    lib_().gasfm_gchain_path_counts(buf)
+    return int(buf[0]), int(buf[1])
+
+
+def fwd(c, tensors, device, stream):
+    sync = _native._counters(device, SYNC_WORDS)
+    return lib_().gasfm_gchain_fwd_fused(ctypes.addressof(c), *(_native._p(t) for t in tensors), _native._p(sync),
+                                         _native._p(status_word(device)), stream)
+
+
+def bwd(c, tensors, d, ws, cnt, device, stream):
+    sync = _native._counters(device, SYNC_WORDS)
+    return lib_().gasfm_gchain_bwd_fused(ctypes.addressof(c), *(_native._p(t) for t in tensors), ctypes.addressof(d),
+                                         _native._p(ws), _native._p(cnt), _native._p(sync),
+                                         _native._p(status_word(device)), stream)
diff --git a/include/gasfm_gchain_fused.h b/include/gasfm_gchain_fused.h
--- /dev/null
+++ b/include/gasfm_gchain_fused.h
@@ -0,0 +1,28 @@
+#ifndef GASFM_GCHAIN_FUSED_H
+#define GASFM_GCHAIN_FUSED_H
+
+#include <stdint.h>
+
+#include "gasfm.h"
+
+#ifdef __cplusplus
+extern "C" {
+#endif
+
+#define GASFM_GCHAIN_SYNC_WORDS 1056
+int gasfm_gchain_fwd_fused(const void* c, const float* xcat, const float* prev, float* x1, float* g,
+                           float* sg, float* xv, float* xp, float* xrv, float* xrp, uint32_t* sync,
+                           uint32_t* status, void* stream);
+int gasfm_gchain_bwd_fused(const void* c, const float* xcat, const float* x1, const float* g,
+                           const float* xv, const float* xp, const float* dskip, const float* dsg,
+                           const float* dxrv, const float* dxrp, float* dxcat, float* dprev,
+                           const void* d, float* scratch, uint32_t* counters, uint32_t* sync,
+                           uint32_t* status, void* stream);
+int gasfm_gchain_fused_set(int32_t on);
+void gasfm_gchain_path_counts(int64_t* out);
+
+#ifdef __cplusplus
+}
+#endif
+
+#endif
```

New measurement: 144.2 million edges/s. No clear change (-0.2%).
